# lucanest/Phyloformer

Hardware: AMD Instinct MI355X
Metric: alignments/sec, 60-leaf/500-site LG+GC-like MSAs, Phyloformer forward (pf.ckpt) (higher is better)
Workload: dtype f16x3-split MFMA (two fp16 limbs per operand, 3 passes), fp32 accumulate/residual

## Files before the change

### phyloformer_amd/csrc/pf_device.hip.h

```cpp
#pragma once
#include <hip/hip_runtime.h>
#include <stdint.h>

#include "pf_layout.h"

namespace pfk {

typedef float f32x4 __attribute__((ext_vector_type(4)));
typedef float f32x16 __attribute__((ext_vector_type(16)));
#if PF_F16
typedef _Float16 h16_t;
#define PF_MFMA(a, b, c) __builtin_amdgcn_mfma_f32_32x32x16_f16((a), (b), (c), 0, 0, 0)
#define PF_DOT2C "v_dot2c_f32_f16"
#define PF_CVT_PK "v_cvt_pk_f16_f32"
#define PF_NEG1_LO 0x0000bc00u
#define PF_NEG1_HI 0xbc000000u
#else
typedef __bf16 h16_t;
#define PF_MFMA(a, b, c) __builtin_amdgcn_mfma_f32_32x32x16_bf16((a), (b), (c), 0, 0, 0)
#define PF_DOT2C "v_dot2c_f32_bf16"
#define PF_CVT_PK "v_cvt_pk_bf16_f32"
#define PF_NEG1_LO 0x0000bf80u
#define PF_NEG1_HI 0xbf800000u
#endif
// ... 152 lines not shown
    r1 = fmaf((float)h2[1], -1.f, g1);
#else
    asm(PF_DOT2C_PRE PF_DOT2C " %0, %2, %4\n\t" PF_DOT2C " %1, %3, %4" PF_DOT2C_POST
                 : "+v"(r0), "+v"(r1) : "s"(PF_NEG1_LO), "s"(PF_NEG1_HI), "v"(hb));
#endif
    const h16x2 l2 = {(h16_t)r0, (h16_t)r1};
    hi_out = hb;
    lo_out = __builtin_bit_cast(unsigned, l2);
}
__device__ __forceinline__ void gelu_split_pair(float x0, float x1, unsigned& hi_out, unsigned& lo_out) {
    split_pair(gelu_scaled(x0), gelu_scaled(x1), hi_out, lo_out);
}
__device__ __forceinline__ void split8(const float* v, frag_t& hi, frag_t& lo) {
#if defined(PF_SPLIT_NODOT) || (PF_F16 && !defined(PF_SPLIT_DOT2C))
    u32x4 h, l;
#pragma unroll
    for (int k = 0; k < 4; ++k) {
        unsigned a, b;
        split_pair(v[2 * k], v[2 * k + 1], a, b);
        h[k] = a;
        l[k] = b;
    }
    hi = __builtin_bit_cast(frag_t, h);
    lo = __builtin_bit_cast(frag_t, l);
#else
    u32x4 h, l;
#pragma unroll
    for (int k = 0; k < 4; ++k) {
        const h16x2 h2 = {(h16_t)v[2 * k], (h16_t)v[2 * k + 1]};
        h[k] = __builtin_bit_cast(unsigned, h2);
    }
    float r0 = v[0], r1 = v[1], r2 = v[2], r3 = v[3], r4 = v[4], r5 = v[5], r6 = v[6], r7 = v[7];
    unsigned l0, l1, l2, l3;
    asm(
        PF_DOT2C " %4, %12, %14\n\t" PF_DOT2C " %5, %13, %14\n\t"
        PF_DOT2C " %6, %12, %15\n\t" PF_DOT2C " %7, %13, %15\n\t"
        PF_DOT2C " %8, %12, %16\n\t" PF_DOT2C " %9, %13, %16\n\t"
        PF_DOT2C " %10, %12, %17\n\t" PF_DOT2C " %11, %13, %17\n\ts_nop 1\n\t"
        PF_CVT_PK " %0, %4, %5\n\t" PF_CVT_PK " %1, %6, %7\n\t" PF_CVT_PK " %2, %8, %9\n\t" PF_CVT_PK " %3, %10, %11"
        : "=&v"(l0), "=&v"(l1), "=&v"(l2), "=&v"(l3),
          "+v"(r0), "+v"(r1), "+v"(r2), "+v"(r3), "+v"(r4), "+v"(r5), "+v"(r6), "+v"(r7)
        : "s"(PF_NEG1_LO), "s"(PF_NEG1_HI), "v"(h[0]), "v"(h[1]), "v"(h[2]), "v"(h[3]));
    l[0] = l0; l[1] = l1; l[2] = l2; l[3] = l3;
    hi = __builtin_bit_cast(frag_t, h);
    lo = __builtin_bit_cast(frag_t, l);
#endif
}
__device__ __forceinline__ void gelu_split8(const f32x16& acc, int base, frag_t& hi, frag_t& lo) {
    float g[8];
#pragma unroll
    for (int k = 0; k < 8; ++k) g[k] = gelu_scaled(acc[base + k]);
    split8(g, hi, lo);
}


__device__ __forceinline__ void mfma3(f32x16& acc, const frag_t& a_hi, const frag_t& a_lo,
                                      const frag_t& b_hi, const frag_t& b_lo, const bool flip = false) {
    if (!flip) {
        acc = PF_MFMA(a_hi, b_lo, acc);
        acc = PF_MFMA(a_hi, b_hi, acc);
        acc = PF_MFMA(a_lo, b_hi, acc);
    } else {
        acc = PF_MFMA(a_lo, b_hi, acc);
        acc = PF_MFMA(a_hi, b_hi, acc);
        acc = PF_MFMA(a_hi, b_lo, acc);
    }
}

__device__ __forceinline__ void mfma3_zero(f32x16& acc, const frag_t& a_hi, const frag_t& a_lo,
                                           const frag_t& b_hi, const frag_t& b_lo, const bool flip = false) {
    const f32x16 z = {0.f, 0.f, 0.f, 0.f, 0.f, 0.f, 0.f, 0.f, 0.f, 0.f, 0.f, 0.f, 0.f, 0.f, 0.f, 0.f};
    if (!flip) {
        acc = PF_MFMA(a_hi, b_lo, z);
        acc = PF_MFMA(a_hi, b_hi, acc);
        acc = PF_MFMA(a_lo, b_hi, acc);
    } else {
        acc = PF_MFMA(a_lo, b_hi, z);
        acc = PF_MFMA(a_hi, b_hi, acc);
        acc = PF_MFMA(a_hi, b_lo, acc);
    }
}

__device__ __forceinline__ void ln_pair(const float (&x)[32], float (&xn)[32]) {
    float s4[4] = {x[0], x[1], x[2], x[3]};
#pragma unroll
    for (int j = 4; j < 32; ++j) s4[j & 3] += x[j];
    const float mean = pair_sum((s4[0] + s4[1]) + (s4[2] + s4[3])) * (1.f / 64.f);
    float v4[4] = {0.f, 0.f, 0.f, 0.f};
#pragma unroll
    for (int j = 0; j < 32; ++j) {
        xn[j] = x[j] - mean;
        v4[j & 3] = fmaf(xn[j], xn[j], v4[j & 3]);
    }
    const float v = (v4[0] + v4[1]) + (v4[2] + v4[3]);
    const float rstd = __builtin_amdgcn_rsqf(pair_sum(v) * (1.f / 64.f) + LN_EPS);
#pragma unroll
    for (int j = 0; j < 32; ++j) xn[j] *= rstd;
}

typedef const f32x4 __attribute__((address_space(3)))* lds_f32x4_t;
__device__ __forceinline__ void load_acc_bias(f32x16& acc, lds_f32_t lds_bias_h) {
#pragma unroll
    for (int q4 = 0; q4 < 4; ++q4) {
        const f32x4 bb = *(lds_f32x4_t)(lds_bias_h + 8 * q4);
#pragma unroll
        for (int i = 0; i < 4; ++i) acc[4 * q4 + i] = bb[i];
    }
}

__device__ __forceinline__ void load_acc_bias(f32x16& acc, const float* lds_bias, int h) {
#pragma unroll
    for (int q4 = 0; q4 < 4; ++q4) {
        const f32x4 bb = *reinterpret_cast<const f32x4*>(lds_bias + 8 * q4 + 4 * h);
#pragma unroll
        for (int i = 0; i < 4; ++i) acc[4 * q4 + i] = bb[i];
    }
}

__device__ __forceinline__ frag_t zero_frag() {
    frag_t z;
#pragma unroll
    for (int i = 0; i < 8; ++i) z[i] = (h16_t)0.f;
    return z;
}

#ifndef PF_DEVICE_HELPERS_ONLY
struct MainArgs {
    float* x;
    float* qrow;
    const float* qcol;
    const frag_t* mfrag;
    const float* rq;
    const float* ctx;
    float* spart;
    float* outpart;
    const frag_t* wimg;
    const float* consts;
    const frag_t* wv_lo;
    const float* table;
    const uint8_t* idx;
    const int16_t* pair_i;
    const int16_t* pair_j;
    int B, N, P, Lloc;
    int flat;
    int nt_aln;
    int slots_aln;
    size_t trash_tok;
    int store_x_last;
    unsigned long long* prof;
    int ablate;
    float* sitemap;
    const float* w;
    const int* srep;
};

enum { MODE_FIRST = 0, MODE_MID = 1, MODE_LAST = 2, MODE_MID0 = 3, MODE_LAST_FOLD = 4 };

struct TilePos { int b, kt, r0, l0; };
template <bool FLAT>
__device__ __forceinline__ TilePos tile_pos(const MainArgs& a, int task, int ntiles) {
    TilePos q;
    q.b = task / a.nt_aln;
    q.kt = task - q.b * a.nt_aln;
    if (FLAT) { const int tok0 = q.kt * 32; q.r0 = tok0 / a.Lloc; q.l0 = tok0 - q.r0 * a.Lloc; }
    else { q.r0 = q.kt / ntiles; q.l0 = (q.kt - q.r0 * ntiles) * 32; }
    return q;
}
template <bool FLAT>
__device__ __forceinline__ TilePos tile_next(const MainArgs& a, TilePos q) {
    if (++q.kt == a.nt_aln) { q.b++; q.kt = 0; q.r0 = 0; q.l0 = 0; return q; }
    q.l0 += 32;
    if (q.l0 >= a.Lloc) { q.l0 = FLAT ? q.l0 - a.Lloc : 0; q.r0++; }
    return q;
}
struct LanePos { size_t tok0; int toff, l, nvalid, wrap; bool valid, in_r1; };
template <bool FLAT>
__device__ __forceinline__ LanePos lane_pos(const MainArgs& a, const TilePos& q, int t) {
    LanePos o;
    o.tok0 = ((size_t)q.b * a.P + q.r0) * a.Lloc + q.l0;
    const int left = FLAT ? a.P * a.Lloc - q.kt * 32 : a.Lloc - q.l0;
    o.nvalid = min(32, left);
    o.wrap = (FLAT && q.r0 + 1 < a.P) ? min(32, a.Lloc - q.l0) : 32;
    o.valid = t < o.nvalid;
    o.toff = min(t, o.nvalid - 1);
    o.in_r1 = o.toff >= o.wrap;
    o.l = q.l0 + o.toff - (o.in_r1 ? a.Lloc : 0);
    return o;
}
__device__ __forceinline__ void part_range(int flat, int pr, int nparts, int P, int L, int slots_aln, long* first, int* count) {
    if (!flat) { *first = (long)pr * nparts; *count = nparts; return; }
    const int b = pr / P, p = pr - b * P;
    const int k0 = (int)(((long)p * L) >> 5), k1 = (int)((((long)p + 1) * L - 1) >> 5);
    *first = (long)b * slots_aln + k0 + p;
    *count = k1 - k0 + 1;
}

template <int LO, int HI>
__device__ __forceinline__ void image_to_lds(const frag_t* src, unsigned char* smem) {
    static_assert(LO % 64 == 0 && HI % 64 == 0, "the image is copied in whole waves");
    const int wv = threadIdx.x >> 6, ln = threadIdx.x & 63;
#pragma unroll
    for (int k = 0; k < (HI - LO + MAIN_THREADS - 1) / MAIN_THREADS; ++k) {
        const int f0 = LO + k * MAIN_THREADS + wv * 64;
        if (f0 < HI) __builtin_amdgcn_global_load_lds(src + f0 + ln, smem + (size_t)f0 * 16, 16, 0, 0);
    }
}

template <int MODE, bool FLAT, bool SITEMAP = false, bool WEIGHTED = false>
__global__ void __launch_bounds__(MAIN_THREADS, MAIN_WAVES / 4) k_main(MainArgs a) {
    constexpr bool LAST = MODE == MODE_LAST || MODE == MODE_LAST_FOLD;
    constexpr bool FOLD = MODE == MODE_LAST_FOLD;
    static_assert(!SITEMAP || LAST, "the site map is the head's: last block only");
    static_assert(!WEIGHTED || (!SITEMAP && MODE != MODE_FIRST), "weighted launches: blocks' own modes, no site map");
    extern __shared__ __attribute__((aligned(16))) unsigned char smem[];
    lds_frag_t lw = (lds_frag_t)smem;
    lds_f32_t lc = (lds_f32_t)(smem + FRAG_END * 16);

    {
        const float cv = a.consts[min((int)threadIdx.x, CONST_LEN - 1)];
        if (FOLD) {
            image_to_lds<FRAG_W1, FRAG_W2>(a.wimg, smem);
            image_to_lds<FRAG_WO, FRAG_U + U_FRAGS>(a.wimg, smem);
        } else {
            image_to_lds<(MODE == MODE_FIRST) ? FRAG_WV : 0, LAST ? FRAG_WV : FRAG_END>(a.wimg, smem);
        }
        static_assert(CONST_LEN <= MAIN_THREADS, "one constant per thread");
        if (threadIdx.x < CONST_LEN) reinterpret_cast<float*>(smem + FRAG_END * 16)[threadIdx.x] = cv;
        asm volatile("s_waitcnt vmcnt(0)" ::: "memory");
    }
    __syncthreads();

    const int lane = threadIdx.x & 63;
    const int wave = __builtin_amdgcn_readfirstlane(threadIdx.x >> 6);
    const int t = lane & 31;
    const int h = lane >> 5;
    const int ntiles = (a.Lloc + 31) >> 5;
    const int ntasks = a.B * a.nt_aln;
    if (wave >= MAIN_WAVES / 2) __builtin_amdgcn_s_setprio(1);
    unsigned long long tacc[6] = {0, 0, 0, 0, 0, 0}, tprev = 0;
#define PF_TICK(k) do { if (a.prof) { const unsigned long long tn_ = __builtin_amdgcn_s_memtime(); tacc[k] += tn_ - tprev; tprev = tn_; } } while (0)
    if (a.prof) tprev = __builtin_amdgcn_s_memtime();
    lds_frag_t w1p = lw + FRAG_W1 + lane;
    lds_frag_t w2p = lw + FRAG_W2 + lane;
    lds_frag_t wop = lw + FRAG_WO + lane;
    lds_frag_t qkp = lw + FRAG_QK + h * 8 + (t & 7);
    lds_f32_t lch = lc + 4 * h;
    PF_OPAQUE(wop); PF_OPAQUE(qkp); PF_OPAQUE(lch);
    lds_frag_t wvp = wop + (FRAG_WV - FRAG_WO);
    lds_f32_t luh = (lds_f32_t)(smem + FRAG_U * 16) + 16 * h;

    {
        const int nwaves = gridDim.x * MAIN_WAVES;
#ifndef PF_RUN_MAX
#define PF_RUN_MAX 8
#endif
        const int run = max(1, min(PF_RUN_MAX, ntasks / (nwaves * 8)));
        int run0 = (blockIdx.x * MAIN_WAVES + wave) * run;
        const int task0 = run0, task1 = ntasks;
        TilePos cur = tile_pos<FLAT>(a, min(task0, ntasks - 1), ntiles);
        int frag_row = -1;
        frag_t mfr[4];
        f32x4 rqv = {0.f, 0.f, 0.f, 0.f};
        f32x4 px[8], pctx[8], pqr, pqc;
        int pri = 0, prj = 0;
        auto prefetch = [&](const TilePos& np) {
            const LanePos nl = lane_pos<FLAT>(a, np, t);
            const int ll = nl.l, pb = np.b;
            const size_t tk = nl.tok0 + nl.toff;
            if (MODE == MODE_MID0) {
                const uint8_t* ib = a.idx + (size_t)pb * a.N * a.Lloc + ll;
                const int pp = np.r0 + (nl.in_r1 ? 1 : 0);
                pri = residue(ib[(size_t)a.pair_i[pp] * a.Lloc]);
                prj = residue(ib[(size_t)a.pair_j[pp] * a.Lloc]);
            } else {
                const f32x4* xp = reinterpret_cast<const f32x4*>(a.x + tk * 64 + 4 * h);
#pragma unroll
                for (int g = 0; g < 8; ++g) px[g] = xp[2 * g];
            }
            pqr = *reinterpret_cast<const f32x4*>(a.qrow + tk * 4);
            pqc = *reinterpret_cast<const f32x4*>(a.qcol + (tk + (size_t)(long)(a.srep[(size_t)pb * a.Lloc + ll] - ll)) * 4);
            if (MODE != MODE_FIRST) {
                int hq = h;
                asm volatile("" : "+v"(hq));
                const f32x4* cp = reinterpret_cast<const f32x4*>(a.ctx + ((size_t)pb * a.Lloc + ll) * 64 + 4 * hq);
#pragma unroll
                for (int g = 0; g < 8; ++g) pctx[g] = cp[2 * g];
            }
        };
        if (MODE != MODE_FIRST && task0 < task1) prefetch(cur);

        for (int task = task0; task < task1;) {
            const int b = cur.b;
            const int row = b * a.P + cur.r0;
            int ntask = task + 1;
            TilePos nxt = tile_next<FLAT>(a, cur);
            if (ntask == run0 + run) {
                run0 += nwaves * run;
                ntask = run0;
                if (ntask < task1) nxt = tile_pos<FLAT>(a, ntask, ntiles);
            }
            const LanePos lp = lane_pos<FLAT>(a, cur, t);
            const bool straddle = lp.wrap < 32;
            int ai = 0, aj = 0;
            if (MODE == MODE_FIRST) { const int pp = cur.r0 + (lp.in_r1 ? 1 : 0); ai = a.pair_i[pp]; aj = a.pair_j[pp]; }
            auto load_mfr = [&](int r) {
                const frag_t* mf = a.mfrag + (size_t)r * 128 + t;
#pragma unroll
                for (int q = 0; q < 4; ++q) mfr[q] = mf[q * 32];
                typedef const f32x4 __attribute__((address_space(4)))* const_f32x4_t;
                rqv = *(const_f32x4_t)(unsigned long long)(a.rq + (size_t)__builtin_amdgcn_readfirstlane(r) * 4);
                frag_row = r;
            };
            if (MODE != MODE_FIRST && row != frag_row) load_mfr(row);
            const bool valid = lp.valid;
            const int lc_ = lp.l;
            const size_t tok = lp.tok0 + lp.toff;
            float x[32];
            float zh[4] = {0.f, 0.f, 0.f, 0.f};
            float wt = 1.f;
            if (WEIGHTED && LAST) wt = a.w[(size_t)b * a.Lloc + lc_];

            if (MODE == MODE_FIRST) {
                const int ri = residue(a.idx[((size_t)b * a.N + ai) * a.Lloc + lc_]);
                const int rj = residue(a.idx[((size_t)b * a.N + aj) * a.Lloc + lc_]);
                const f32x4* ti = reinterpret_cast<const f32x4*>(a.table + ri * 64 + 4 * h);
                const f32x4* tj = reinterpret_cast<const f32x4*>(a.table + rj * 64 + 4 * h);
#pragma unroll
                for (int g = 0; g < 8; ++g) {
                    f32x4 u = ti[2 * g], w = tj[2 * g];
#pragma unroll
                    for (int i = 0; i < 4; ++i) x[4 * g + i] = u[i] + w[i];
                }
            } else {
                if (MODE == MODE_MID0) {
                    const f32x4* ti = reinterpret_cast<const f32x4*>(a.table + pri * 64 + 4 * h);
                    const f32x4* tj = reinterpret_cast<const f32x4*>(a.table + prj * 64 + 4 * h);
#pragma unroll
                    for (int g = 0; g < 8; ++g) {
                        const f32x4 u = ti[2 * g], w = tj[2 * g];
#pragma unroll
                        for (int i = 0; i < 4; ++i) x[4 * g + i] = u[i] + w[i];
                    }
                } else {
#pragma unroll
                    for (int g = 0; g < 8; ++g)
#pragma unroll
                        for (int i = 0; i < 4; ++i) x[4 * g + i] = px[g][i];
                }
                PF_TICK(0);
                if (!(a.ablate & 8)) {
                    f32x16 ya[2];
#pragma unroll
                    for (int j = 0; j < 32; ++j) ya[j >> 4][j & 15] = x[j];
                    {
                        const f32x4 qr = pqr;
                        auto mix = [&](const bool mine) {
                            float v[8];
#pragma unroll
                            for (int i = 0; i < 4; ++i) v[i] = mine ? qr[i] * rqv[i] : 0.f;
                            v[4] = v[5] = mine ? 1.f : 0.f;
                            v[6] = v[7] = 0.f;
                            frag_t qb_hi, qb_lo;
                            split8(v, qb_hi, qb_lo);
#pragma unroll
                            for (int To = 0; To < 2; ++To) mfma3(ya[To], mfr[To * 2], mfr[To * 2 + 1], qb_hi, qb_lo, To == 1);
                        };
                        mix(h == 0 && !lp.in_r1);
                        if (straddle) {
                            load_mfr(row + 1);
                            mix(h == 0 && lp.in_r1);
                        }
                    }
                    {
                        const f32x4 qc = pqc * COLAPPLY_B_SCALE;
                        float o[32];
#pragma unroll
                        for (int g = 0; g < 8; ++g) {
                            const f32x4 u = pctx[g];
#pragma unroll
                            for (int i = 0; i < 4; ++i) o[4 * g + i] = u[i] * qc[g >> 1];
                        }
#pragma unroll
                        for (int s = 0; s < 4; ++s) {
                            frag_t ob_hi, ob_lo;
                            split8(&o[8 * s], ob_hi, ob_lo);
#pragma unroll
                            for (int To = 0; To < 2; ++To) {
                                lds_frag_t f = wop + ((To * 4 + s) * 2) * 64;
                                const frag_t a_hi = f[0], a_lo = f[64];
                                mfma3(ya[To], a_hi, a_lo, ob_hi, ob_lo, To == 1);
                            }
                        }
                    }
#pragma unroll
                    for (int j = 0; j < 32; ++j) x[j] = ya[j >> 4][j & 15];
                }

                PF_TICK(1);
                if (FOLD) {
#pragma unroll
                    for (int g = 0; g < 8; ++g) {
                        const f32x4 w4 = *(lds_f32x4_t)(lch + CONST_HW + 8 * g);
#pragma unroll
                        for (int i = 0; i < 4; ++i) zh[i] = fmaf(w4[i], x[4 * g + i], zh[i]);
                    }
                }
                if (FOLD && !(a.ablate & 16)) {
                    frag_t xb_hi[4], xb_lo[4];
                    {
                        float xn[32];
                        ln_pair(x, xn);
#pragma unroll
                        for (int s = 0; s < 4; ++s) split8(&xn[8 * s], xb_hi[s], xb_lo[s]);
                    }
                    if (ntask < task1) prefetch(nxt);
                    PF_TICK(2);
#pragma unroll 1
                    for (int T = 0; T < 8; ++T) {
                        f32x16 ha;
                        lds_frag_t f1 = w1p + T * 512;
                        lds_f32_t bp = lch + CONST_B1 + 32 * T;
                        lds_f32_t up = luh + 32 * T;
                        PF_OPAQUE(f1); PF_OPAQUE(bp); PF_OPAQUE(up);
                        load_acc_bias(ha, bp);
                        frag_t fh = f1[0], fl = f1[64];
#pragma unroll
                        for (int s = 0; s < 4; ++s) {
                            frag_t nh = fh, nl = fl;
                            if (s < 3) { nh = f1[(s + 1) * 128]; nl = f1[(s + 1) * 128 + 64]; }
                            mfma3(ha, fh, fl, xb_hi[s], xb_lo[s]);
                            fh = nh; fl = nl;
                        }
#pragma unroll
                        for (int q = 0; q < 4; ++q) {
                            const f32x4 u4 = *(lds_f32x4_t)(up + 4 * q);
#pragma unroll
                            for (int i = 0; i < 4; ++i) zh[i] = fmaf(u4[i], gelu_scaled(ha[4 * q + i]), zh[i]);
                        }
                    }
                    PF_TICK(3);
                } else if (!(a.ablate & 16)) {
                    frag_t xb_hi[4], xb_lo[4];
                    {
                        float xn[32];
                        ln_pair(x, xn);
#pragma unroll
                        for (int s = 0; s < 4; ++s) split8(&xn[8 * s], xb_hi[s], xb_lo[s]);
                    }
                    f32x16 oa[2];
                    load_acc_bias(oa[0], lch + CONST_B2);
                    load_acc_bias(oa[1], lch + CONST_B2 + 32);
#pragma unroll
                    for (int j = 0; j < 32; ++j) oa[j >> 4][j & 15] += x[j];
                    if (ntask < task1) prefetch(nxt);
                    PF_TICK(2);
#pragma unroll 1
                    for (int T = 0; T < 8; ++T) {
                        f32x16 ha;
                        lds_frag_t f1 = w1p + T * 512;
                        lds_frag_t f2 = w2p + T * 256;
                        lds_f32_t bp = lch + CONST_B1 + 32 * T;
                        PF_OPAQUE(f1); PF_OPAQUE(f2); PF_OPAQUE(bp);
                        load_acc_bias(ha, bp);
                        frag_t fh = f1[0], fl = f1[64];
#pragma unroll
                        for (int s = 0; s < 4; ++s) {
                            frag_t nh, nl;
                            if (s < 3) { nh = f1[(s + 1) * 128]; nl = f1[(s + 1) * 128 + 64]; }
                            else { nh = f2[0]; nl = f2[64]; }
                            mfma3(ha, fh, fl, xb_hi[s], xb_lo[s]);
                            fh = nh; fl = nl;
                        }
                        frag_t g_hi[2], g_lo[2];
                        gelu_split8(ha, 0, g_hi[0], g_lo[0]);
                        gelu_split8(ha, 8, g_hi[1], g_lo[1]);
#pragma unroll
                        for (int st = 0; st < 4; ++st) {
                            const int u = st >> 1, To = st & 1;
                            frag_t nh = fh, nl = fl;
                            if (st < 3) {
                                const int nu = (st + 1) >> 1, nTo = (st + 1) & 1;
                                nh = f2[(nTo * 32 + nu * 2) * 64];
                                nl = f2[(nTo * 32 + nu * 2) * 64 + 64];
                            }
                            mfma3(oa[To], fh, fl, g_hi[u], g_lo[u], To == 1);
                            fh = nh; fl = nl;
                        }
                    }
                    PF_TICK(3);
#pragma unroll
                    for (int j = 0; j < 32; ++j) x[j] = oa[j >> 4][j & 15];
                }
            }

            if (!LAST && !(a.ablate & 4)) {
                frag_t wl[8];
#pragma unroll
                for (int i = WVLO_LDS; i < 8; ++i) wl[i] = a.wv_lo[i * 64 + lane];
                if (WEIGHTED) wt = a.w[(size_t)b * a.Lloc + lc_];
                __builtin_amdgcn_sched_barrier(0);
                {
                    const size_t stok = valid ? tok : a.trash_tok + t;
                    f32x4* xo = reinterpret_cast<f32x4*>(a.x + stok * 64 + 4 * h);
#pragma unroll
                    for (int g = 0; g < 8; ++g) {
                        f32x4 u = {x[4 * g], x[4 * g + 1], x[4 * g + 2], x[4 * g + 3]};
                        xo[2 * g] = u;
                    }
                }
                if (a.ablate & 32) { cur = nxt; task = ntask; continue; }
                f32x16 va[3];
                {
                    float xn[32];
                    ln_pair(x, xn);
                    frag_t xb_hi[4], xb_lo[4];
#pragma unroll
                    for (int s = 0; s < 4; ++s) split8(&xn[8 * s], xb_hi[s], xb_lo[s]);
#pragma unroll
                    for (int s = 0; s < 4; ++s) {
                        const frag_t q_hi = qkp[(s * 2) * 16], q_lo = qkp[(s * 2 + 1) * 16];
                        if (s == 0) mfma3_zero(va[2], q_hi, q_lo, xb_hi[s], xb_lo[s]);
                        else mfma3(va[2], q_hi, q_lo, xb_hi[s], xb_lo[s]);
                    }
#pragma unroll
                    for (int s = 0; s < 4; ++s)
#pragma unroll
                        for (int T = 0; T < 2; ++T) {
                            const frag_t f_hi = wvp[(T * 4 + s) * 64];
                            const frag_t f_lo = T * 4 + s < WVLO_LDS ? wvp[(FRAG_WVLO - FRAG_WV) + (T * 4 + s) * 64] : wl[T * 4 + s];
                            if (s == 0) mfma3_zero(va[T], f_hi, f_lo, xb_hi[s], xb_lo[s], T == 1);
                            else mfma3(va[T], f_hi, f_lo, xb_hi[s], xb_lo[s], T == 1);
                        }
                }
#pragma unroll
                for (int r = 0; r < 4; ++r) va[2][r] += lc[CONST_BQK + 4 * h + r];
                float qk[4], ot[4];
#pragma unroll
                for (int i = 0; i < 4; ++i) qk[i] = elu1_fast(va[2][i]);
#pragma unroll
                for (int i = 0; i < 4; ++i) ot[i] = pair_other(qk[i], h);
                float qn[4], kn[4];
#pragma unroll
                for (int i = 0; i < 4; ++i) {
                    qn[i] = h ? ot[i] : qk[i];
                    kn[i] = h ? qk[i] : ot[i];
                }
                {
                    const size_t stok = valid ? tok : a.trash_tok + t;
                    f32x4 qs = {qn[0], qn[1], qn[2], qn[3]};
                    *reinterpret_cast<f32x4*>(a.qrow + stok * 4) = qs;
                }
                const long slot0 = (long)b * a.slots_aln + cur.kt + (FLAT ? cur.r0 : 0);
                for (int part = 0; part < (straddle ? 2 : 1); ++part) {
                    float* sp = a.spart + (size_t)(slot0 + part) * SROW;
                    const float vm = (valid && lp.in_r1 == (part == 1)) ? (WEIGHTED ? wt : 1.f) : 0.f;
                    float km[4];
#pragma unroll
                    for (int i = 0; i < 4; ++i) km[i] = kn[i] * vm;
                    {
                        float qk8[8];
#pragma unroll
                        for (int i = 0; i < 4; ++i) { qk8[i] = vm * qn[i]; qk8[4 + i] = km[i]; }
                        const float sqk = treduce8(qk8, t);
                        if (lane < 8) sp[64 + lane] = sqk;
                    }
                    {
                        float kv[32];
#pragma unroll
                        for (int j = 0; j < 32; ++j) kv[j] = km[j >> 3] * va[j >> 4][j & 15];
                        sp[kmap(t, h)] = treduce32(kv, t);
                    }
                }
            } else if (LAST) {
                float z = 0.f;
                if (FOLD) {
                    z = pair_sum((zh[0] + zh[1]) + (zh[2] + zh[3])) + lc[CONST_C0];
                } else {
#pragma unroll
                    for (int g = 0; g < 8; ++g) {
                        const f32x4 w4 = *(lds_f32x4_t)(lch + CONST_HW + 8 * g);
#pragma unroll
                        for (int i = 0; i < 4; ++i) z = fmaf(w4[i], x[4 * g + i], z);
                    }
                    z = pair_sum(z) + lc[CONST_HB];
                }
                const float spz = softplus20(z);
                const long slot0 = (long)b * a.slots_aln + cur.kt + (FLAT ? cur.r0 : 0);
                for (int part = 0; part < (straddle ? 2 : 1); ++part) {
                    const float so = half32_sum((valid && lp.in_r1 == (part == 1)) ? (WEIGHTED ? wt * spz : spz) : 0.f);
                    if (lane == 0) a.outpart[slot0 + part] = so;
                }
                if (SITEMAP && valid && h == 0) a.sitemap[lp.tok0 + lp.toff] = spz;
                if (!FOLD && a.store_x_last && valid) {
                    f32x4* xo = reinterpret_cast<f32x4*>(a.x + tok * 64 + 4 * h);
#pragma unroll
                    for (int g = 0; g < 8; ++g) {
                        f32x4 u = {x[4 * g], x[4 * g + 1], x[4 * g + 2], x[4 * g + 3]};
                        xo[2 * g] = u;
                    }
                }
            }
            PF_TICK(4);
            cur = nxt;
            task = ntask;
        }
    }
    if (a.prof && __builtin_amdgcn_mbcnt_hi(~0u, __builtin_amdgcn_mbcnt_lo(~0u, 0u)) == 0) {
#pragma unroll
        for (int k = 0; k < 6; ++k) atomicAdd(a.prof + k, tacc[k]);
    }
#undef PF_TICK
}

constexpr int EMBED_THREADS = 512;
constexpr int EMBED_LDS_BYTES = (PAIRTAB_ROWS * PAIRTAB_W + 22 * 64) * 4;
struct EmbedArgs {
    const uint8_t* idx;
    const int16_t* pair_i;
    const int16_t* pair_j;
    const float* ptab;
    const float* table;
    float* x;
    float* qrow;
    float* srow;
    int B, N, P, Lloc;
    unsigned* bad_idx;
    const float* w;
};

template <bool WEIGHTED = false>
__global__ void __launch_bounds__(EMBED_THREADS) k_embed(EmbedArgs a) {
    extern __shared__ __attribute__((aligned(16))) float esm[];
    float* tab = esm;
    float* emb = esm + PAIRTAB_ROWS * PAIRTAB_W;
    {
        constexpr int NV = PAIRTAB_ROWS * PAIRTAB_W / 4, FULL = NV / EMBED_THREADS;
        const f32x4* src = reinterpret_cast<const f32x4*>(a.ptab);
        f32x4* dst = reinterpret_cast<f32x4*>(tab);
        const int wv = threadIdx.x >> 6, ln = threadIdx.x & 63;
#pragma unroll
        for (int k = 0; k < FULL; ++k) {
            const int v0 = k * EMBED_THREADS + wv * 64;
            __builtin_amdgcn_global_load_lds(src + v0 + ln, tab + (size_t)v0 * 4, 16, 0, 0);
        }
        const int it = FULL * EMBED_THREADS + threadIdx.x;
        const f32x4 tail = src[min(it, NV - 1)];
        const f32x4* s2 = reinterpret_cast<const f32x4*>(a.table);
        f32x4* d2 = reinterpret_cast<f32x4*>(emb);
        static_assert(22 * 64 / 4 <= EMBED_THREADS, "one embedding vector per thread");
        const f32x4 ev = s2[min((int)threadIdx.x, 22 * 64 / 4 - 1)];
        if (it < NV) dst[it] = tail;
        if (threadIdx.x < 22 * 64 / 4) d2[threadIdx.x] = ev;
        asm volatile("s_waitcnt vmcnt(0)" ::: "memory");
    }
    __syncthreads();
    const int lane = threadIdx.x & 63, wave = threadIdx.x >> 6;
    const int sg = lane >> 4, cl = lane & 15;
    const int ntasks = a.B * a.P;
    for (int task = blockIdx.x * (EMBED_THREADS / 64) + wave; task < ntasks; task += gridDim.x * (EMBED_THREADS / 64)) {
        const int b = task / a.P, p = task - b * a.P;
        const uint8_t* ri = a.idx + ((size_t)b * a.N + a.pair_i[p]) * a.Lloc;
        const uint8_t* rj = a.idx + ((size_t)b * a.N + a.pair_j[p]) * a.Lloc;
        const size_t row0 = (size_t)task * a.Lloc;
        f32x4 acc = {0.f, 0.f, 0.f, 0.f}, acce = {0.f, 0.f, 0.f, 0.f};
        bool bad = false;
        auto fetch = [&](int blk) {
            const int l = min(blk * 64 + lane, a.Lloc - 1);
            const int ra = ri[l], rb = rj[l];
            bad |= max(ra, rb) >= NA;
            return residue(ra) * 22 + residue(rb);
        };
        auto fetch_w = [&](int blk) { return WEIGHTED ? a.w[(size_t)b * a.Lloc + min(blk * 64 + lane, a.Lloc - 1)] : 1.f; };
        const int nblk = (a.Lloc + 63) >> 6;
        int cur = fetch(0);
        float wcur = fetch_w(0);
        for (int blk = 0; blk < nblk; ++blk) {
            const int nxt = fetch(min(blk + 1, nblk - 1));
            const float wnxt = fetch_w(min(blk + 1, nblk - 1));
            const int lbase = blk * 64;
            const int nit = min(16, (a.Lloc - lbase + 3) >> 2);
            auto site = [&](int it, bool valid) {
                const int l = lbase + 4 * it + sg;
                const int rr = __shfl(cur, 4 * it + sg);
                const float* tr = tab + rr * PAIRTAB_W;
                const f32x4 s = *reinterpret_cast<const f32x4*>(tr + 4 * cl);
                const f32x4 e = *reinterpret_cast<const f32x4*>(tr + 64 + 4 * (cl & 1));
                const float wl = WEIGHTED ? __shfl(wcur, 4 * it + sg) : 1.f;
                if (valid) {
                    if (WEIGHTED) {
                        acc += wl * s;
                        acce += wl * e;
                    } else {
                        acc += s;
                        acce += e;
                    }
                    const size_t tok = row0 + l;
                    if (a.x) {
                        const int ra = rr / 22, rb = rr - 22 * ra;
                        const f32x4 xa = *reinterpret_cast<const f32x4*>(emb + ra * 64 + 4 * cl);
                        const f32x4 xb = *reinterpret_cast<const f32x4*>(emb + rb * 64 + 4 * cl);
                        *reinterpret_cast<f32x4*>(a.x + tok * 64 + 4 * cl) = xa + xb;
                    }
                    if (cl == 0) *reinterpret_cast<f32x4*>(a.qrow + tok * 4) = e;
                }
            };
            if (lbase + 64 <= a.Lloc) {
#pragma unroll 4
                for (int it = 0; it < 16; ++it) site(it, true);
            } else {
                for (int it = 0; it < nit; ++it) site(it, lbase + 4 * it + sg < a.Lloc);
            }
            cur = nxt;
            wcur = wnxt;
        }
#pragma unroll
        for (int i = 0; i < 4; ++i) {
            acc[i] += __shfl_xor(acc[i], 16);
            acc[i] += __shfl_xor(acc[i], 32);
            acce[i] += __shfl_xor(acce[i], 16);
            acce[i] += __shfl_xor(acce[i], 32);
        }
        if (sg == 0) {
            float* sr = a.srow + (size_t)task * SROW;
            *reinterpret_cast<f32x4*>(sr + 4 * cl) = acc;
            if (cl < 2) *reinterpret_cast<f32x4*>(sr + 64 + 4 * cl) = acce;
        }
        if (bad && a.bad_idx) *a.bad_idx = 1u;
    }
}

struct RowFinArgs {
    const float* srow;
    float* mrow;
    frag_t* mfrag;
    const float* woT;
    const float* bv;
    const float* bias;
    const float* bias_col;
    int npairs, nparts;
    float L_total;
    int flat, P, Lloc, slots_aln;
    int iters;
    float* rq;
    float a_scale, b_scale;
    const float* wst;
};

__global__ void __launch_bounds__(256) k_rowfin(RowFinArgs a) {
    __shared__ float ctx[4][64];
    __shared__ float mm[4][6][64];
    __shared__ float st[4][SROW];
    __shared__ float rqs[4][4];
    const int sub = threadIdx.x >> 6, c = threadIdx.x & 63;
    float wo[4][16];
#pragma unroll
    for (int hh = 0; hh < 4; ++hh)
#pragma unroll
        for (int d = 0; d < 16; ++d) wo[hh][d] = a.woT[(16 * hh + d) * 64 + c];
    const float bvc = a.bv[c], biasc = a.bias[c], biascol = a.bias_col[c];
    for (int it = 0; it < a.iters; ++it) {
    const int pr = (blockIdx.x * a.iters + it) * 4 + sub;
    const bool ok = pr < a.npairs;
    if (ok) {
        long first;
        int nparts;
        part_range(a.flat, pr, a.nparts, a.P, a.Lloc, a.slots_aln, &first, &nparts);
        const float* sp = a.srow + (size_t)first * SROW;
        const int c2 = 64 + (c & 7);
        float acc = 0.f, acc2 = 0.f;
        for (int i = 0; i < nparts; i += 8) {
            const float* q0 = sp + i * SROW;
            float v[8], w8[8];
#pragma unroll
            for (int q = 0; q < 8; ++q) {
                const bool on = i + q < nparts;
                v[q] = on ? q0[q * SROW + c] : 0.f;
                w8[q] = on ? q0[q * SROW + c2] : 0.f;
            }
#pragma unroll
            for (int q = 0; q < 8; ++q) { acc += v[q]; acc2 += w8[q]; }
        }
        st[sub][c] = acc;
        if (c < 8) st[sub][64 + c] = acc2;
    }
    __syncthreads();
    if (ok) {
        const float* s = st[sub];
        const int hh = c >> 4;
        const float sk = s[68 + hh];
        ctx[sub][c] = (s[c] + bvc * sk) / sk;
        if (c < 4) {
            const float* ws = a.wst ? a.wst + (size_t)(pr / a.P) * 4 : nullptr;
            const float r = (ws ? ws[0] : a.L_total) / s[64 + c];
            rqs[sub][c] = r;
            a.rq[(size_t)pr * 4 + c] = r * (ws ? ws[2] : a.b_scale);
        }
    }
    __syncthreads();
    if (ok) {
        float* m = a.mrow ? a.mrow + (size_t)pr * MROW : nullptr;
#pragma unroll
        for (int hh = 0; hh < 4; ++hh) {
            float acc = 0.f;
#pragma unroll
            for (int d = 0; d < 16; ++d) acc = fmaf(wo[hh][d], ctx[sub][16 * hh + d], acc);
            if (m) m[hh * 64 + c] = acc * rqs[sub][hh];
            mm[sub][hh][c] = acc * (a.wst ? a.wst[(size_t)(pr / a.P) * 4 + 3] : a.a_scale);
        }
        mm[sub][4][c] = biasc;
        mm[sub][5][c] = biascol;
    }
    __syncthreads();
    if (ok) {
        const int To = c >> 5, t = c & 31;
        float v[8];
#pragma unroll
        for (int i = 0; i < 8; ++i) v[i] = (i < 6) ? mm[sub][i][32 * To + t] : 0.f;
        frag_t hi, lo;
        split8(v, hi, lo);
        frag_t* mf = a.mfrag + (size_t)pr * MFRAG_PER_PAIR + To * 64 + t;
        mf[0] = hi;
        mf[32] = lo;
    }
    }
}

__global__ void k_rowsum(const float* spart, float* srow, int npairs, int nparts_, int flat, int P, int Lloc, int slots_aln) {
    const int i = blockIdx.x * blockDim.x + threadIdx.x;
    if (i >= npairs * SROW) return;
    const int pr = i / SROW, c = i - pr * SROW;
    long first;
    int nparts;
    part_range(flat, pr, nparts_, P, Lloc, slots_aln, &first, &nparts);
    const float* sp = spart + (size_t)first * SROW + c;
    float acc = 0.f;
    for (int k = 0; k < nparts; k += 8) {
        float v[8];
#pragma unroll
        for (int q = 0; q < 8; ++q) v[q] = k + q < nparts ? sp[(size_t)(k + q) * SROW] : 0.f;
#pragma unroll
        for (int q = 0; q < 8; ++q) acc += v[q];
    }
    srow[i] = acc;
}

__global__ void k_outsum(const float* outpart, float* out, int npairs, int nparts_, float inv_L_total, int flat, int P,
                         int Lloc, int slots_aln, const float* wst) {
    const int pr = blockIdx.x * blockDim.x + threadIdx.x;
    if (pr >= npairs) return;
    long first;
    int nparts;
    part_range(flat, pr, nparts_, P, Lloc, slots_aln, &first, &nparts);
    const float* sp = outpart + first;
    float acc = 0.f;
    for (int k = 0; k < nparts; k += 8) {
        float v[8];
#pragma unroll
        for (int q = 0; q < 8; ++q) v[q] = k + q < nparts ? sp[k + q] : 0.f;
#pragma unroll
        for (int q = 0; q < 8; ++q) acc += v[q];
    }
    out[pr] = acc * (wst ? wst[(size_t)(pr / P) * 4 + 1] : inv_L_total);
}

struct SiteClassArgs {
    const uint8_t* idx;
    int* srep;
    int* ulist;
    int* ucount;
    int N, Lloc, dedup;
};
constexpr int SC_THREADS = 1024, SC_MAX_SITES = 4096;
__global__ void __launch_bounds__(SC_THREADS) k_site_classes(SiteClassArgs a) {
    __shared__ __attribute__((aligned(16))) uint32_t hsh[SC_MAX_SITES];
    __shared__ int wsum[SC_THREADS / 64];
    const int b = blockIdx.x, tid = threadIdx.x, lane = tid & 63, wave = tid >> 6;
    const uint8_t* ib = a.idx + (size_t)b * a.N * a.Lloc;
    int* const srep = a.srep + (size_t)b * a.Lloc;
    int* const ulist = a.ulist + (size_t)b * a.Lloc;
    const bool dedup = a.dedup && a.Lloc <= SC_MAX_SITES;
    auto same_column = [&](int c, int l) {
        unsigned diff = 0;
#pragma unroll 8
        for (int n = 0; n < a.N; ++n) diff |= (unsigned)(ib[(size_t)n * a.Lloc + c] ^ ib[(size_t)n * a.Lloc + l]);
        return diff == 0;
    };
    if (dedup) {
        for (int l = tid; l < a.Lloc; l += SC_THREADS) {
            uint32_t hv = 0x811C9DC5u;
#pragma unroll 8
            for (int n = 0; n < a.N; ++n) hv = (hv ^ ib[(size_t)n * a.Lloc + l]) * 0x01000193u;
            hsh[l] = hv;
        }
        __syncthreads();
    }
    int base = 0;
    for (int l0 = 0; l0 < a.Lloc; l0 += SC_THREADS) {
        const int l = l0 + tid;
        int rep = l;
        if (dedup && l < a.Lloc) {
            const uint32_t mine = hsh[l];
            int cand = l;
            for (int c0 = 0; c0 < l && cand == l; c0 += 4) {
                const u32x4 v = *reinterpret_cast<const u32x4*>(hsh + c0);
#pragma unroll
                for (int i = 3; i >= 0; --i)
                    if (v[i] == mine && c0 + i < l) cand = c0 + i;
            }
            if (cand < l) {
                if (same_column(cand, l)) rep = cand;
                else
                    for (int c = cand + 1; c < l && rep == l; ++c)
                        if (hsh[c] == mine && same_column(c, l)) rep = c;
            }
        }
        const bool first = l < a.Lloc && rep == l;
        if (l < a.Lloc) srep[l] = rep;
        const unsigned long long m = __ballot(first);
        if (lane == 0) wsum[wave] = __popcll(m);
        __syncthreads();
        int before = 0, total = 0;
#pragma unroll
        for (int w = 0; w < SC_THREADS / 64; ++w) { const int n = wsum[w]; total += n; if (w < wave) before += n; }
        if (first) ulist[base + before + __popcll(m & ((1ull << lane) - 1ull))] = l;
        base += total;
        __syncthreads();
    }
    if (tid == 0) a.ucount[b] = base;
}

struct ColStatsArgs {
    const float* x;
    const float* qrow;
    const float* mrow;
    float* qcol;
    float* part;
    const float* wqk;
    const float* bqk;
    const float* brow;
    int B, P, Lloc, G, nchunks;
    int sub, S, fine;
    const float* table;
    const uint8_t* idx;
    const int16_t* pair_i;
    const int16_t* pair_j;
    int N;
    const int* ulist;
    const int* ucount;
};
constexpr int CPART = 4 * 64 + 8;

constexpr int CS_SLOT = 2 * 256 + 64;
#ifndef PF_CS_RING
#define PF_CS_RING 4
#endif
#ifndef PF_CS_MT
#define PF_CS_MT 16
#endif
template <bool EMBED, int RING, int MT>
#ifndef PF_CS_WAVES
#define PF_CS_WAVES 2
#endif
__global__ void __launch_bounds__(256, PF_CS_WAVES) k_colstats(ColStatsArgs a) {
    static_assert(!(EMBED && RING), "block 0 reads residue bytes, not x");
    static_assert(RING % 2 == 0, "pairs are consumed two at a time");
    static_assert(MT == 16 || MT == 8, "pair matrices are staged 16 or 8 at a time (runs are multiples of 8)");
    constexpr int LDS_MST = 2 * MT * MROW, LDS_RING = RING ? 4 * RING * CS_SLOT : 0, LDS_EMB = EMBED ? 22 * 64 : 0;
    constexpr int PIJ_CAP = 640;
    __shared__ __attribute__((aligned(16))) float lds_all[LDS_MST + LDS_RING + LDS_EMB + (EMBED ? PIJ_CAP : 0)];
    int bid = blockIdx.x;
    int run = 0;
    if (a.fine) { run = bid % a.S; bid /= a.S; }
    const int g = bid % a.G; bid /= a.G;
    const int chunk = bid % a.nchunks;
    const int b = bid / a.nchunks;
    const int nu = a.ucount[b];
    if (chunk * 32 >= nu) return;
    const int* const ul = a.ulist + (size_t)b * a.Lloc;
    float* const mst = lds_all;
    float* const xring = lds_all + LDS_MST;
    float* const emb = lds_all + LDS_MST + LDS_RING;
    int16_t* const pij = reinterpret_cast<int16_t*>(lds_all + LDS_MST + LDS_RING + LDS_EMB);
    if (EMBED) {
        constexpr int NV = 22 * 64 / 4;
        const f32x4* tsrc = reinterpret_cast<const f32x4*>(a.table);
        const int i0 = threadIdx.x, i1 = threadIdx.x + 256;
        static_assert(NV <= 2 * 256, "two vectors per thread cover the table");
        const f32x4 v0 = tsrc[min(i0, NV - 1)], v1 = tsrc[min(i1, NV - 1)];
        if (i0 < NV) reinterpret_cast<f32x4*>(emb)[i0] = v0;
        if (i1 < NV) reinterpret_cast<f32x4*>(emb)[i1] = v1;
    }
    const int lane = threadIdx.x & 63, wave = threadIdx.x >> 6;
    const int ts = lane >> 3, cl = lane & 7;
    const int per = (a.P + a.G - 1) / a.G;

    f32x2 w2[4][8];
#pragma unroll
    for (int o = 0; o < 8; o += 2)
#pragma unroll
        for (int q = 0; q < 2; ++q) {
            const f32x4 u0 = *reinterpret_cast<const f32x4*>(a.wqk + o * 64 + 8 * cl + 4 * q);
            const f32x4 u1 = *reinterpret_cast<const f32x4*>(a.wqk + (o + 1) * 64 + 8 * cl + 4 * q);
#pragma unroll
            for (int i = 0; i < 4; ++i) w2[o >> 1][4 * q + i] = f32x2{u0[i], u1[i]};
        }
    const float bj = a.bqk[cl];
    const f32x4 br0 = *reinterpret_cast<const f32x4*>(a.brow + 8 * cl), br1 = *reinterpret_cast<const f32x4*>(a.brow + 8 * cl + 4);
    const bool up1 = (cl & 2) != 0, up0 = (cl & 1) != 0;
    const int us = chunk * 32 + wave * 8 + ts;
    const bool lvalid = us < nu;
    const int l = ul[min(us, nu - 1)];
    const int lcl = l;
    const int gp0 = g * per, gp1 = min(a.P, gp0 + per);
    const int p0 = a.fine ? gp0 + run * a.sub : gp0, p1 = a.fine ? min(gp1, p0 + a.sub) : gp1;
    if (p0 >= p1) return;
    const float vmask = lvalid ? 1.f : 0.f;
    f32x2 z[4][4], zt[4][4];
// ... 342 lines not shown
```

### phyloformer_amd/csrc/pf_layout.h

```cpp
#pragma once

#ifndef PF_F16
#define PF_F16 1
#endif

namespace pfk {

constexpr int E = 64;
constexpr int NH = 4;
constexpr int HD = 16;
constexpr int FF = 256;
constexpr int NA = 22;
constexpr int SROW = 72;
constexpr int MROW = 4 * 64;
constexpr float LN_EPS = 1e-5f;

constexpr int FRAG_W1 = 0;
constexpr int FRAG_W2 = FRAG_W1 + 8 * 4 * 2 * 64;
constexpr int FRAG_WO = FRAG_W2 + 2 * 16 * 2 * 64;
constexpr int FRAG_WV = FRAG_WO + 2 * 4 * 2 * 64;
constexpr int FRAG_QK = FRAG_WV + 2 * 4 * 64;
#ifndef PF_WVLO_LDS
#define PF_WVLO_LDS 4
#endif
constexpr int WVLO_LDS = PF_WVLO_LDS;
constexpr int FRAG_WVLO = FRAG_QK + 4 * 2 * 16;
constexpr int FRAG_END = FRAG_WVLO + WVLO_LDS * 64;
constexpr int FRAG_U = FRAG_WV;
constexpr int U_FRAGS = FF * 4 / 16;
static_assert(FRAG_U + U_FRAGS <= FRAG_END, "the folded head fits the last block's tail");
constexpr int WVLO_FRAGS = 2 * 4 * 64;
constexpr int CONST_B1 = 0, CONST_B2 = 256, CONST_BQK = 320, CONST_HW = 328, CONST_HB = 392,
              CONST_C0 = 393, CONST_BOC = 400;
constexpr int CONST_LEN = 464;
constexpr int MAIN_LDS_BYTES = FRAG_END * 16 + CONST_LEN * 4;
constexpr int MFRAG_PER_PAIR = 2 * 2 * 32;

constexpr int MAIN_THREADS = 512;
constexpr int MAIN_WAVES = MAIN_THREADS / 64;

constexpr int PAIRTAB_ROWS = 22 * 22, PAIRTAB_W = 72;

}
```

### phyloformer_amd/csrc/pf_lib.hip

```cpp
#include <hip/hip_runtime.h>
#include <dlfcn.h>

#include <algorithm>
#include <cmath>
#include <cstdarg>
#include <cstdio>
#include <cstdlib>
#include <cstring>
#include <functional>
#include <map>
#include <mutex>
#include <string>
#include <type_traits>
#include <vector>

#include "../../include/phyloformer_amd.h"
#include "pf_device.hip.h"
#include "pf_mha.hip.h"
#include "pf_precise.hip.h"
#include "pf_generic.hip.h"
#include "pf_boot.hip.h"
#include "pf_sites.hip.h"
#include "pf_sitemap.hip.h"
#include "pf_sites_host.h"
// ... 15 lines not shown

namespace {

thread_local std::string g_create_error;

struct PfNcclId { char internal[128]; };
struct RcclApi {
    void* lib = nullptr;
    int (*GetUniqueId)(void*) = nullptr;
    int (*CommInitRank)(void**, int, PfNcclId, int) = nullptr;
    int (*AllReduce)(const void*, void*, size_t, int, int, void*, hipStream_t) = nullptr;
    int (*CommDestroy)(void*) = nullptr;
    const char* (*GetErrorString)(int) = nullptr;
};
RcclApi g_rccl;
std::string g_rccl_path;
int g_rccl_version = 0;
std::once_flag g_rccl_once;
std::string g_rccl_err;

bool load_rccl_once(std::string& err) {
    std::vector<std::string> names;
    if (const char* env = std::getenv("PF_RCCL_LIB")) names.push_back(env);
    else {
        if (const char* rocm = std::getenv("ROCM_PATH")) names.push_back(std::string(rocm) + "/lib/librccl.so.1");
        names.push_back("/opt/rocm/lib/librccl.so.1");
        names.push_back("librccl.so.1");
        names.push_back("librccl.so");
    }
    void* lib = nullptr;
    std::string tried;
    for (const std::string& n : names) {
        lib = dlopen(n.c_str(), RTLD_NOW | RTLD_LOCAL);
        if (lib) break;
        tried += (tried.empty() ? "" : ", ") + n;
    }
    if (!lib) { err = "cannot load librccl (tried " + tried + "): " + dlerror(); return false; }
    g_rccl.GetUniqueId = reinterpret_cast<int (*)(void*)>(dlsym(lib, "ncclGetUniqueId"));
    g_rccl.CommInitRank = reinterpret_cast<int (*)(void**, int, PfNcclId, int)>(dlsym(lib, "ncclCommInitRank"));
    g_rccl.AllReduce = reinterpret_cast<int (*)(const void*, void*, size_t, int, int, void*, hipStream_t)>(
        dlsym(lib, "ncclAllReduce"));
    g_rccl.CommDestroy = reinterpret_cast<int (*)(void*)>(dlsym(lib, "ncclCommDestroy"));
    g_rccl.GetErrorString = reinterpret_cast<const char* (*)(int)>(dlsym(lib, "ncclGetErrorString"));
    if (!g_rccl.GetUniqueId || !g_rccl.CommInitRank || !g_rccl.AllReduce || !g_rccl.CommDestroy) {
        err = "librccl is missing required symbols";
        return false;
    }
    Dl_info rinfo{}, hinfo{}, mine{};
    dladdr(reinterpret_cast<void*>(g_rccl.GetUniqueId), &rinfo);
    g_rccl_path = rinfo.dli_fname ? rinfo.dli_fname : "?";
    void* rccl_hip = dlsym(lib, "hipGetDeviceCount");
    if (rccl_hip && dladdr(rccl_hip, &hinfo) && dladdr(reinterpret_cast<void*>(&hipGetDeviceCount), &mine) &&
        hinfo.dli_fname && mine.dli_fname && std::strcmp(hinfo.dli_fname, mine.dli_fname) != 0) {
        err = std::string("librccl (") + g_rccl_path + ") is bound to the HIP runtime " + hinfo.dli_fname +
              " but this library uses " + mine.dli_fname + "; set PF_RCCL_LIB to the matching librccl";
        dlclose(lib);
        return false;
    }
    if (auto getv = reinterpret_cast<int (*)(int*)>(dlsym(lib, "ncclGetVersion"))) getv(&g_rccl_version);
    g_rccl.lib = lib;
    return true;
}
bool load_rccl(std::string& err) {
    std::call_once(g_rccl_once, [] { if (!load_rccl_once(g_rccl_err) && g_rccl_err.empty()) g_rccl_err = "librccl unavailable"; });
    if (g_rccl.lib) return true;
    err = g_rccl_err;
    return false;
}
constexpr int NCCL_FLOAT = 7, NCCL_DOUBLE = 8, NCCL_SUM = 0;

struct BlockDev {
    float* wimg = nullptr;
    float* consts = nullptr;
    float* wv_lo = nullptr;
    float* bqk_row = nullptr;
    float* row_woT = nullptr;
    float* row_bv = nullptr;
    float* row_bo = nullptr;
    float* col_bo = nullptr;
    float* col_wqk = nullptr;
    float* col_bqk = nullptr;
    float* col_wvT = nullptr;
    float* col_bv = nullptr;
};

struct ProfSlot { int kid; hipEvent_t a, b; };
const char* const KNAMES[] = {"embed", "rowfin", "colstats", "colfin", "main", "allreduce",
                              "mha_qkv", "mha_attn", "mha_out", "precise", "generic", "resample", "gather", "site_moments", "gather_taxa", "loo_stats",
                              "weight_sums", "place_stats", "tile_combine", "bme_pairs", "site_classes"};
enum { K_EMBED = 0, K_ROWFIN, K_COLSTATS, K_COLFIN, K_MAIN, K_ALLREDUCE, K_MHA_QKV, K_MHA_ATTN, K_MHA_OUT, K_PRECISE, K_GENERIC,
       K_RESAMPLE, K_GATHER, K_SITE_MOMENTS, K_GATHER_TAXA, K_LOO_STATS, K_WEIGHT_SUMS, K_PLACE_STATS, K_TILE_COMBINE, K_BME_PAIRS, K_SITE_CLASSES, K_COUNT };

struct F64Ends {
    const double* table = nullptr;
    const double *hw = nullptr, *hb = nullptr;
};

struct PreciseWeights {
    F64Ends ends;
    double* blob = nullptr;
    std::vector<pfp::AttnW> row, col;
    std::vector<pfp::FfnW> ffn;
};

struct GenericWeights {
    F64Ends ends;
    bool ready = false;
    std::vector<pfg::AttnW> row, col;
    std::vector<pfg::FfnW> ffn;
};

constexpr int64_t SUB_FLOATS_DEFAULT = (int64_t)1 << 22;

struct DeviceBuffer {
    void* p = nullptr; size_t cap = 0;
    explicit DeviceBuffer(std::vector<DeviceBuffer*>& all) { all.push_back(this); }
    DeviceBuffer(const DeviceBuffer&) = delete;
    int reserve(pf_handle* h, size_t bytes);
    void release() { if (p) hipFree(p); p = nullptr; cap = 0; }
};
template <class T> struct Buffer : DeviceBuffer {
    using DeviceBuffer::DeviceBuffer;
    operator T*() const { return static_cast<T*>(p); }
};

}

struct pf_handle {
    int device = 0;
    int n_blocks = 0;
    hipStream_t stream = nullptr;
    hipStream_t stream2 = nullptr;
    hipStream_t cur = nullptr;
    hipEvent_t ev_fork = nullptr, ev_join = nullptr;
    hipDeviceProp_t prop;
    std::string err;
    int64_t max_seqs = 200;
    bool profile = false;
    bool profile_main_only = false;
    bool debug_keep = false;
    int ablate = 0;
    unsigned long long* phase_prof = nullptr;
    bool phase_prof_last = false;
    bool head_fold = true;
    bool force_rccl = false;
    int64_t ws_limit_bytes = (int64_t)24 << 30;
    float* table = nullptr;
    float* pair_table = nullptr;
    bool embed_mfma = false;
    int colstats_fine = -1;
    bool colstats_ring = true;
    bool materialize_x0 = false;
    bool site_dedup = true;
    float* first_consts = nullptr;
    float* first_img = nullptr;
    std::vector<BlockDev> blk;
    std::vector<void*> owned;
    std::vector<DeviceBuffer*> buffers;
    int pair_n = -1;
    Buffer<int16_t> pair_i{buffers}, pair_j{buffers};
    Buffer<char> ws{buffers}, ws2{buffers};
    bool overlap = true;
    int reserve_cus = 8;
    Buffer<uint8_t> d_idx{buffers};
    Buffer<float> d_out{buffers};
    Buffer<uint8_t> d_rep{buffers};
    Buffer<int32_t> d_map{buffers};
    Buffer<float> d_smap{buffers}, d_se{buffers}, d_prof{buffers};
    Buffer<double> d_mpart{buffers};
    Buffer<char> d_sub{buffers};
    int64_t sub_floats = SUB_FLOATS_DEFAULT;
    pftile::Plan tiled_plan;
    pftile::Tables tiled_tab;
    Buffer<char> d_tiled_tab{buffers};
    Buffer<char> d_nj{buffers}, d_nj_io{buffers};
    int64_t nj_calls = 0;
    int64_t bionj_calls = 0;
    Buffer<char> d_delta_io{buffers};
    int64_t delta_calls = 0;
    bool delta_atomic = true;
    Buffer<char> d_bme{buffers};
    Buffer<float> d_bme_preds{buffers};
    int64_t bme_calls = 0;
    int64_t spr_calls = 0;
    bool spr_pairs_simple = false;
    int64_t spr_step_cap = 0;
    Buffer<char> d_sup{buffers}, d_sup_io{buffers};
    Buffer<uint8_t> d_sup_bad{buffers};
    int64_t sup_calls = 0;
    int64_t transfer_calls = 0;
    Buffer<char> d_con{buffers}, d_con_io{buffers};
    int64_t con_calls = 0;
    Buffer<float> d_w{buffers}, d_wst{buffers}, d_wtab{buffers};
    void* comm[2] = {nullptr, nullptr};
    int rank = 0, world = 1;
    int64_t coll_calls = 0;
    bool sharded_call = false;
    bool reducing = false;
    bool two_streams = true;
    std::vector<ProfSlot> pending;
    std::vector<hipEvent_t> free_events;
    int64_t prof_n[K_COUNT] = {0};
    double prof_ms[K_COUNT] = {0};
    std::map<std::string, std::vector<float>> taps;
    int tile_force = -1;
    int precise = -1;
    double recheck_above = 8.0;
    int64_t rechecked = 0;
    bool f16_ok = true;
    double f16_vmax_col = 0.0;
    char f16_why[160] = {0};
    bool precise_ffn_valu = false;
    PreciseWeights pw;
    Buffer<char> wsp{buffers};
    bool arch_generic = false;
    int generic = 0;
    pfg::Arch garch{};
    GenericWeights gw;
    std::vector<float> blob_copy;
    unsigned* bad_idx_host = nullptr;
    unsigned* bad_idx_dev = nullptr;
};

namespace {

int fail(pf_handle* h, int code, const char* fmt, ...) {
    char buf[512];
    va_list ap;
    va_start(ap, fmt);
    vsnprintf(buf, sizeof buf, fmt, ap);
    va_end(ap);
    if (h) h->err = buf; else g_create_error = buf;
    return code;
}

#define HIPCHK(h, call)                                                                 \
    do {                                                                                \
        hipError_t e_ = (call);                                                         \
        if (e_ != hipSuccess)                                                           \
            return fail((h), e_ == hipErrorOutOfMemory ? PF_ENOMEM : PF_EHIP, "%s: %s", \
                        #call, hipGetErrorString(e_));                                  \
    } while (0)

template <typename T>
int upload(pf_handle* h, const std::vector<T>& v, float** out) {
    void* p = nullptr;
    HIPCHK(h, hipMalloc(&p, v.size() * sizeof(T)));
    h->owned.push_back(p);
    HIPCHK(h, hipMemcpy(p, v.data(), v.size() * sizeof(T), hipMemcpyHostToDevice));
    *out = reinterpret_cast<float*>(p);
    return PF_OK;
}

int DeviceBuffer::reserve(pf_handle* h, size_t bytes) {
    if (p && bytes <= cap) return PF_OK;
    hipError_t e = hipSuccess;
    if (p) {
        e = hipStreamSynchronize(h->stream);
        if (e == hipSuccess && h->stream2) e = hipStreamSynchronize(h->stream2);
        release();
    }
    if (e == hipSuccess && (e = hipMalloc(&p, bytes ? bytes : 1)) != hipSuccess) p = nullptr;
    if (e != hipSuccess)
        return fail(h, e == hipErrorOutOfMemory ? PF_ENOMEM : PF_EHIP, "device buffer of %zu bytes: %s", bytes, hipGetErrorString(e));
    cap = bytes;
    return PF_OK;
}

struct F16Ranges { double hidden = 0, mbase = 0, vmax_col = 0, wmax = 0; };
void f16_note_attn(const std::vector<float>& wv, const std::vector<float>& bv, const float* wo, bool col, F16Ranges* r) {
    double vmax[E];
    for (int hd = 0; hd < E; ++hd) {
        double n2 = 0;
        for (int c = 0; c < E; ++c) { n2 += (double)wv[(size_t)hd * E + c] * wv[(size_t)hd * E + c]; r->wmax = std::max(r->wmax, std::fabs((double)wv[(size_t)hd * E + c])); }
        vmax[hd] = std::sqrt(n2) * 8.0 + std::fabs((double)bv[hd]);
        if (col) r->vmax_col = std::max(r->vmax_col, vmax[hd]);
    }
    for (int c = 0; c < E; ++c)
        for (int hh = 0; hh < NH; ++hh) {
            double m = 0;
            for (int d = 0; d < HD; ++d) { m += std::fabs((double)wo[(size_t)c * E + 16 * hh + d]) * vmax[16 * hh + d]; r->wmax = std::max(r->wmax, std::fabs((double)wo[(size_t)c * E + 16 * hh + d]) * (col ? COLAPPLY_A_SCALE : 1.0)); }
            if (!col) r->mbase = std::max(r->mbase, m);
        }
}
void f16_note_ffn(const std::vector<float>& w1a, const std::vector<float>& b1a, const std::vector<float>& w2s, F16Ranges* r) {
    for (int j = 0; j < FF; ++j) {
        double n2 = 0;
        for (int c = 0; c < E; ++c) { n2 += (double)w1a[(size_t)j * E + c] * w1a[(size_t)j * E + c]; r->wmax = std::max(r->wmax, std::fabs((double)w1a[(size_t)j * E + c])); }
        r->hidden = std::max(r->hidden, 2.0 * (std::sqrt(n2) * 8.0 + std::fabs((double)b1a[j])));
    }
    for (float v : w2s) r->wmax = std::max(r->wmax, std::fabs((double)v));
}
constexpr double F16_LIMIT = 60000.0;
void check_f16_ranges(pf_handle* h, const F16Ranges& r) {
    h->f16_vmax_col = r.vmax_col;
    const bool finite = std::isfinite(r.hidden) && std::isfinite(r.mbase) && std::isfinite(r.vmax_col) && std::isfinite(r.wmax);
    h->f16_ok = !PF_F16 || (finite && r.hidden < F16_LIMIT && r.mbase * 64.0 < F16_LIMIT && r.wmax < F16_LIMIT);
    if (!h->f16_ok)
        snprintf(h->f16_why, sizeof h->f16_why, "fp16 operand bounds: hidden %.3g, row-mix base %.3g, weights %.3g (limit %.0f)",
                 r.hidden, r.mbase * 64.0, r.wmax, F16_LIMIT);
}
bool f16_range_ok(const pf_handle* h, int N, int L_total) {
    if (!PF_F16) return true;
    const double P = (double)N * (N - 1) / 2;
    return h->f16_ok && P * h->f16_vmax_col * COLAPPLY_B_SCALE < F16_LIMIT && L_total <= (1 << 20);
}

int prepare_weights(pf_handle* h, const BlobView& view, uint64_t blob_len) {
    if ((uint64_t)view.len != blob_len)
        return fail(h, PF_EINVAL, "weight blob has %llu floats, expected %llu",
                    (unsigned long long)blob_len, (unsigned long long)view.len);
    std::vector<float> table((size_t)NA * E);
    build_embed_table(view, E, E, table.data());
    int rc = upload(h, table, &h->table);
    if (rc) return rc;

    const int nb = (int)view.ffn.size();
    h->blk.resize(nb);

    {
        std::vector<float> ptab;
        build_pair_table(table.data(), view.row[0], ptab);
        if ((rc = upload(h, ptab, &h->pair_table))) return rc;
    }
    F16Ranges ranges;
    std::vector<std::vector<float>> row_bqk(nb);
    std::vector<std::vector<uint16_t>> row_tail(nb);
    for (int k = 0; k < nb; ++k) {
        BlockDev& d = h->blk[k];
        const AttnHost& r = view.row[k];
        const AttnHost& c = view.col[k];
        std::vector<float> wq, bq, wk, bk, wv, bv;
        fold(r.wq, r.bq, r.g, r.b, NH, E, wq, bq);
        fold(r.wk, r.bk, r.g, r.b, NH, E, wk, bk);
        fold(r.wv, r.bv, r.g, r.b, E, E, wv, bv);
        f16_note_attn(wv, bv, r.wo, false, &ranges);
        for (float v : wq) ranges.wmax = std::max(ranges.wmax, std::fabs((double)v));
        for (float v : wk) ranges.wmax = std::max(ranges.wmax, std::fabs((double)v));
        row_tail[k].assign((size_t)(FRAG_END - FRAG_WV) * 8, 0);
        std::vector<uint16_t> wvlo((size_t)WVLO_FRAGS * 8);
        pack_row_stats(wv.data(), wq.data(), wk.data(), row_tail[k].data(), wvlo.data());
        std::copy(wvlo.begin(), wvlo.begin() + (size_t)WVLO_LDS * 64 * 8, row_tail[k].begin() + (size_t)(FRAG_WVLO - FRAG_WV) * 8);
        if ((rc = upload(h, wvlo, &d.wv_lo))) return rc;
        row_bqk[k].assign(8, 0.f);
        for (int i = 0; i < 4; ++i) { row_bqk[k][i] = bq[i]; row_bqk[k][4 + i] = bk[i]; }
        std::vector<float> woT((size_t)E * E);
        for (int cc = 0; cc < E; ++cc)
            for (int hd = 0; hd < E; ++hd) woT[(size_t)hd * E + cc] = r.wo[(size_t)cc * E + hd];
        if ((rc = upload(h, woT, &d.row_woT))) return rc;
        if ((rc = upload(h, bv, &d.row_bv))) return rc;
        if ((rc = upload(h, std::vector<float>(r.bo, r.bo + E), &d.row_bo))) return rc;
        if ((rc = upload(h, std::vector<float>(c.bo, c.bo + E), &d.col_bo))) return rc;
        std::vector<float> cwq, cbq, cwk, cbk, cwv, cbv;
        fold(c.wq, c.bq, c.g, c.b, NH, E, cwq, cbq);
        fold(c.wk, c.bk, c.g, c.b, NH, E, cwk, cbk);
        fold(c.wv, c.bv, c.g, c.b, E, E, cwv, cbv);
        f16_note_attn(cwv, cbv, c.wo, true, &ranges);
        std::vector<float> wqk((size_t)8 * E), bqk(8);
        std::copy(cwq.begin(), cwq.end(), wqk.begin());
        std::copy(cwk.begin(), cwk.end(), wqk.begin() + 4 * E);
        for (int i = 0; i < 4; ++i) { bqk[i] = cbq[i]; bqk[4 + i] = cbk[i]; }
        if ((rc = upload(h, wqk, &d.col_wqk))) return rc;
        if ((rc = upload(h, bqk, &d.col_bqk))) return rc;
        std::vector<float> wvT((size_t)E * E);
        for (int hd = 0; hd < E; ++hd)
            for (int cc = 0; cc < E; ++cc) wvT[(size_t)cc * E + hd] = cwv[(size_t)hd * E + cc];
        if ((rc = upload(h, wvT, &d.col_wvT))) return rc;
        if ((rc = upload(h, cbv, &d.col_bv))) return rc;
    }
    for (int k = 0; k < nb; ++k) {
        BlockDev& d = h->blk[k];
        const FfnHost& f = view.ffn[k];
        std::vector<float> w1f, b1f;
        fold(f.w1, f.b1, f.g, f.b, FF, E, w1f, b1f);
        const double alpha = std::sqrt(0.5 * 1.4426950408889634074);
        for (auto& v : w1f) v = (float)((double)v * alpha);
        for (auto& v : b1f) v = (float)((double)v * alpha);
        std::vector<float> w2s((size_t)E * FF);
        for (size_t i = 0; i < w2s.size(); ++i) w2s[i] = (float)((double)f.w2[i] / alpha * 0.5);
        f16_note_ffn(w1f, b1f, w2s, &ranges);
        std::vector<uint16_t> img((size_t)FRAG_END * 8);
        pack_frags(w1f.data(), FF, E, FF, img.data() + (size_t)FRAG_W1 * 8);
        pack_frags(w2s.data(), E, FF, E, img.data() + (size_t)FRAG_W2 * 8);
        pack_frags(view.col[k].wo, E, E, E, img.data() + (size_t)FRAG_WO * 8, COLAPPLY_A_SCALE);
        if (k + 1 < nb) std::copy(row_tail[k + 1].begin(), row_tail[k + 1].end(), img.begin() + (size_t)FRAG_WV * 8);
        float c0 = 0.f;
        if (k + 1 == nb) {
            float u[FF];
            fold_head(f.w2, f.b2, view.head_w, view.head_b[0], 1.0 / alpha * 0.5, u, &c0);
            std::memcpy(img.data() + (size_t)FRAG_U * 8, u, sizeof(u));
        }
        if ((rc = upload(h, img, &d.wimg))) return rc;
        std::vector<float> cst(CONST_LEN, 0.f);
        std::copy(b1f.begin(), b1f.end(), cst.begin() + CONST_B1);
        std::copy(f.b2, f.b2 + E, cst.begin() + CONST_B2);
        if (k + 1 < nb) std::copy(row_bqk[k + 1].begin(), row_bqk[k + 1].end(), cst.begin() + CONST_BQK);
        std::copy(view.head_w, view.head_w + E, cst.begin() + CONST_HW);
        cst[CONST_HB] = view.head_b[0];
        cst[CONST_C0] = c0;
        std::copy(view.col[k].bo, view.col[k].bo + E, cst.begin() + CONST_BOC);
        if ((rc = upload(h, cst, &d.consts))) return rc;
    }
    std::vector<float> cst0(CONST_LEN, 0.f);
    std::copy(row_bqk[0].begin(), row_bqk[0].end(), cst0.begin() + CONST_BQK);
    std::vector<uint16_t> img0((size_t)FRAG_END * 8, 0);
    std::copy(row_tail[0].begin(), row_tail[0].end(), img0.begin() + (size_t)FRAG_WV * 8);
    check_f16_ranges(h, ranges);
    if ((rc = upload(h, img0, &h->first_img))) return rc;
    return upload(h, cst0, &h->first_consts);
}

int ensure_pairs(pf_handle* h, int N) {
    if (h->pair_n == N) return PF_OK;
    const int P = N * (N - 1) / 2;
    std::vector<int16_t> pi(P), pj(P);
    int k = 0;
    for (int i = 0; i < N; ++i)
        for (int j = i + 1; j < N; ++j) { pi[k] = (int16_t)i; pj[k] = (int16_t)j; ++k; }
    h->pair_n = -1;
    int rc = h->pair_i.reserve(h, P * sizeof(int16_t));
    if (rc || (rc = h->pair_j.reserve(h, P * sizeof(int16_t)))) return rc;
    HIPCHK(h, hipMemcpyAsync(h->pair_i, pi.data(), P * sizeof(int16_t), hipMemcpyHostToDevice, h->stream));
    HIPCHK(h, hipMemcpyAsync(h->pair_j, pj.data(), P * sizeof(int16_t), hipMemcpyHostToDevice, h->stream));
    HIPCHK(h, hipStreamSynchronize(h->stream));
    h->pair_n = N;
    return PF_OK;
}

size_t align_up(size_t v, size_t a) { return (v + a - 1) / a * a; }

TilePlan tile_plan(const pf_handle* h, int P, int Lloc) { return tile_plan_core(P, Lloc, h->tile_force); }

struct Workspace {
    float *x, *qrow, *qcol, *srow, *mrow, *part, *ctx, *mfrag, *spart, *outpart, *rq;
    int *srep, *ulist, *ucount;
    int G;
    int sub, S, fine;
    int nparts() const { return fine ? G * S : G; }
};
constexpr int WS_BUFS = 12;

size_t workspace_bytes(const pf_handle* h, int B, int P, int Lloc, Workspace* w, size_t off[WS_BUFS]) {
    Lloc = std::max(Lloc, 1);
    const ColPlan c = colstats_plan_core(B, P, Lloc, h->colstats_fine);
    w->G = c.G; w->sub = c.sub; w->S = c.S; w->fine = c.fine;
    const int nparts = w->nparts();
    const size_t tok = (size_t)B * P * Lloc;
    size_t o = 0;
    off[0] = o; o = align_up(o + (tok + 32) * 64 * 4, 256);
    off[1] = o; o = align_up(o + (tok + 32) * 4 * 4, 256);
    off[2] = o; o = align_up(o + (tok + 32) * 4 * 4, 256);
    off[3] = o; o = align_up(o + (size_t)B * P * SROW * 4, 256);
    off[4] = o; o = align_up(o + (size_t)B * P * MROW * 4, 256);
    off[5] = o; o = align_up(o + (size_t)B * nparts * Lloc * CPART * 4, 256);
    off[6] = o; o = align_up(o + (size_t)B * Lloc * 64 * 4, 256);
    off[7] = o; o = align_up(o + (size_t)B * P * MFRAG_PER_PAIR * 16, 256);
    const size_t slots = (size_t)tile_plan(h, P, Lloc).slots_aln;
    off[8] = o; o = align_up(o + (size_t)B * slots * SROW * 4, 256);
    off[9] = o; o = align_up(o + (size_t)B * slots * 4, 256);
    off[10] = o; o = align_up(o + (size_t)B * P * 4 * 4, 256);
    off[11] = o; o = align_up(o + ((size_t)B * Lloc * 2 + B) * sizeof(int), 256);
    return o;
}
void carve_workspace(char* ws, const size_t off[WS_BUFS], Workspace* w, int B, int Lloc) {
    w->x = (float*)(ws + off[0]); w->qrow = (float*)(ws + off[1]);
    w->qcol = (float*)(ws + off[2]); w->srow = (float*)(ws + off[3]);
    w->mrow = (float*)(ws + off[4]); w->part = (float*)(ws + off[5]);
    w->ctx = (float*)(ws + off[6]);
    w->mfrag = (float*)(ws + off[7]);
    w->spart = (float*)(ws + off[8]); w->outpart = (float*)(ws + off[9]);
    w->rq = (float*)(ws + off[10]);
    const size_t nsite = (size_t)B * std::max(Lloc, 1);
    w->srep = (int*)(ws + off[11]); w->ulist = w->srep + nsite; w->ucount = w->ulist + nsite;
}

int ensure_workspace(pf_handle* h, int B, int P, int Lloc, Workspace* w, bool second = false) {
    size_t off[WS_BUFS];
    const size_t need = workspace_bytes(h, B, P, Lloc, w, off);
    Buffer<char>& ws = second ? h->ws2 : h->ws;
    if (const int rc = ws.reserve(h, need)) return rc;
    carve_workspace(ws, off, w, B, Lloc);
    return PF_OK;
}

hipEvent_t get_event(pf_handle* h) {
    if (!h->free_events.empty()) { hipEvent_t e = h->free_events.back(); h->free_events.pop_back(); return e; }
    hipEvent_t e;
    hipEventCreate(&e);
    return e;
}
struct ProfScope {
    pf_handle* h; int kid; hipEvent_t a{}, b{};
    bool on;
    ProfScope(pf_handle* h_, int kid_) : h(h_), kid(kid_) {
        on = h->profile && (!h->profile_main_only || kid_ == K_MAIN);
        if (on) { a = get_event(h); b = get_event(h); hipEventRecord(a, h->cur); }
    }
    ~ProfScope() {
        if (on) { hipEventRecord(b, h->cur); h->pending.push_back({kid, a, b}); }
    }
};
void drain_profile(pf_handle* h) {
    if (h->pending.empty()) return;
    hipStreamSynchronize(h->stream);
    if (h->stream2) hipStreamSynchronize(h->stream2);
    for (auto& s : h->pending) {
        float ms = 0.f;
        if (hipEventElapsedTime(&ms, s.a, s.b) == hipSuccess) { h->prof_n[s.kid]++; h->prof_ms[s.kid] += ms; }
        h->free_events.push_back(s.a);
        h->free_events.push_back(s.b);
    }
    h->pending.clear();
}

int save_tap(pf_handle* h, const std::string& name, const float* dptr, size_t n) {
    std::vector<float>& v = h->taps[name];
    v.resize(n);
    HIPCHK(h, hipStreamSynchronize(h->cur));
    HIPCHK(h, hipMemcpy(v.data(), dptr, n * sizeof(float), hipMemcpyDeviceToHost));
    return PF_OK;
}

int allreduce(pf_handle* h, void* buf, size_t count, int dtype = NCCL_FLOAT) {
    if (!h->sharded_call) return PF_OK;
    if (h->world <= 1 && !h->comm[0]) return PF_OK;
    if (!h->comm[0]) return fail(h, PF_ESTATE, "sharded forward on %d ranks needs pf_comm_init", h->world);
    ProfScope ps(h, K_ALLREDUCE);
    void* comm = h->comm[(h->cur == h->stream2 && h->stream2) ? 1 : 0];
    ++h->coll_calls;
    int rc = g_rccl.AllReduce(buf, buf, count, dtype, NCCL_SUM, comm, h->cur);
    if (rc != 0)
        return fail(h, PF_ERCCL, "ncclAllReduce failed: %s",
                    g_rccl.GetErrorString ? g_rccl.GetErrorString(rc) : "?");
    return PF_OK;
}

template <int MODE, bool SITEMAP = false, bool WEIGHTED = false>
int launch_main(pf_handle* h, const MainArgs& a, int kid) {
    const long ntasks = (long)a.B * a.nt_aln;
    const int cus = std::max(1, h->prop.multiProcessorCount - (h->reducing ? h->reserve_cus : 0));
    const int grid = (int)std::max<long>(1, std::min<long>(cus, (ntasks + MAIN_WAVES - 1) / MAIN_WAVES));
    ProfScope ps(h, kid);
    if (a.flat) hipLaunchKernelGGL((k_main<MODE, true, SITEMAP, WEIGHTED>), dim3(grid), dim3(MAIN_THREADS), MAIN_LDS_BYTES, h->cur, a);
    else hipLaunchKernelGGL((k_main<MODE, false, SITEMAP, WEIGHTED>), dim3(grid), dim3(MAIN_THREADS), MAIN_LDS_BYTES, h->cur, a);
    HIPCHK(h, hipGetLastError());
    return PF_OK;
}

struct RowStats { const float* p; int nparts; int flat; };
struct ShardRun {
    Workspace w;
    const uint8_t* d_idx;
    float* d_out;
    int B, N, P, Lloc, L_total;
    TilePlan tp;
    hipStream_t stream;
    RowStats rs;
    float* d_smap = nullptr;
    const float* d_w = nullptr;
    const float* d_wst = nullptr;
};

int zero_fill(pf_handle* h, float* p, size_t n) {
    HIPCHK(h, hipMemsetAsync(p, 0, n * sizeof(float), h->cur));
    return PF_OK;
}

MainArgs main_args(pf_handle* h, const ShardRun& r) {
    MainArgs m{};
    m.x = r.w.x; m.qrow = r.w.qrow; m.qcol = r.w.qcol;
    m.mfrag = reinterpret_cast<const frag_t*>(r.w.mfrag); m.rq = r.w.rq; m.ctx = r.w.ctx; m.spart = r.w.spart;
    m.outpart = r.w.outpart; m.table = h->table; m.idx = r.d_idx; m.pair_i = h->pair_i; m.pair_j = h->pair_j;
    m.B = r.B; m.N = r.N; m.P = r.P; m.Lloc = r.Lloc;
    m.flat = r.tp.flat; m.nt_aln = r.tp.nt_aln; m.slots_aln = r.tp.slots_aln;
    m.store_x_last = h->debug_keep ? 1 : 0;
    m.trash_tok = (size_t)r.B * r.P * r.Lloc;
    m.ablate = h->ablate;
    m.prof = h->phase_prof_last ? nullptr : h->phase_prof;
    m.w = r.d_w;
    m.srep = r.w.srep;
    return m;
}

bool x0_on_the_fly(const pf_handle* h) {
    return !h->materialize_x0 && !h->embed_mfma && h->n_blocks > 1;
}

int launch_site_classes(pf_handle* h, const uint8_t* d_idx, int B, int N, int Lloc, int* srep, int* ulist, int* ucount) {
    if (!Lloc) return PF_OK;
    SiteClassArgs a{d_idx, srep, ulist, ucount, N, Lloc, h->site_dedup ? 1 : 0};
    ProfScope ps(h, K_SITE_CLASSES);
    hipLaunchKernelGGL(k_site_classes, dim3(B), dim3(SC_THREADS), 0, h->cur, a);
    HIPCHK(h, hipGetLastError());
    return PF_OK;
}

int phase_first(pf_handle* h, const ShardRun& r) {
    if (!r.Lloc) return zero_fill(h, r.w.srow, (size_t)r.B * r.P * SROW);
    int rc;
    if (h->embed_mfma) {
        MainArgs m = main_args(h, r);
        m.wimg = reinterpret_cast<const frag_t*>(h->first_img); m.consts = h->first_consts;
        m.wv_lo = reinterpret_cast<const frag_t*>(h->blk[0].wv_lo);
        rc = launch_main<MODE_FIRST>(h, m, K_EMBED);
        if (rc) return rc;
    } else {
        float* x0 = (x0_on_the_fly(h) && !h->debug_keep) ? nullptr : r.w.x;
        EmbedArgs e{r.d_idx, h->pair_i, h->pair_j, h->pair_table, h->table, x0, r.w.qrow, r.w.srow,
                    r.B, r.N, r.P, r.Lloc, h->bad_idx_dev, r.d_w};
        const int ntasks = r.B * r.P, wpb = EMBED_THREADS / 64;
        const int grid = std::max(1, std::min(h->prop.multiProcessorCount, (ntasks + wpb - 1) / wpb));
        ProfScope ps(h, K_EMBED);
        if (r.d_w) hipLaunchKernelGGL(k_embed<true>, dim3(grid), dim3(EMBED_THREADS), EMBED_LDS_BYTES, h->cur, e);
        else hipLaunchKernelGGL(k_embed<false>, dim3(grid), dim3(EMBED_THREADS), EMBED_LDS_BYTES, h->cur, e);
        HIPCHK(h, hipGetLastError());
    }
    if (h->debug_keep) return save_tap(h, "x0", r.w.x, (size_t)r.B * r.P * r.Lloc * 64);
    return PF_OK;
}

int tiles_of(int Lloc) { return (Lloc + 31) / 32; }

int launch_rowsum(pf_handle* h, const ShardRun& r, RowStats* rs) {
    if (rs->p == r.w.srow) return PF_OK;
    const int n = r.B * r.P * SROW;
    if (!r.Lloc) { *rs = RowStats{r.w.srow, 1, 0}; return zero_fill(h, r.w.srow, n); }
    ProfScope ps(h, K_ROWFIN);
    hipLaunchKernelGGL(k_rowsum, dim3((n + 255) / 256), dim3(256), 0, h->cur, rs->p, r.w.srow, r.B * r.P, rs->nparts,
                       rs->flat, r.P, r.Lloc, r.tp.slots_aln);
    HIPCHK(h, hipGetLastError());
    *rs = RowStats{r.w.srow, 1, 0};
    return PF_OK;
}

int launch_outsum(pf_handle* h, const ShardRun& r) {
    const int n = r.B * r.P;
    if (!r.Lloc) return zero_fill(h, r.d_out, n);
    ProfScope ps(h, K_ROWFIN);
    const TilePlan& tp = r.tp;
    hipLaunchKernelGGL(k_outsum, dim3((n + 255) / 256), dim3(256), 0, h->cur, r.w.outpart, r.d_out, n,
                       tiles_of(r.Lloc), 1.0f / (float)r.L_total, tp.flat, r.P, r.Lloc, tp.slots_aln, r.d_wst);
    HIPCHK(h, hipGetLastError());
    return PF_OK;
}

RowStats main_stats(const ShardRun& r) { return RowStats{r.w.spart, tiles_of(r.Lloc), r.tp.flat}; }

RowStats first_stats(pf_handle* h, const ShardRun& r) {
    return h->embed_mfma ? main_stats(r) : RowStats{r.w.srow, 1, 0};
}

int phase_block(pf_handle* h, const ShardRun& r, int k, RowStats rs) {
    if (!r.Lloc) return PF_OK;
    const BlockDev& d = h->blk[k];
    const Workspace& w = r.w;
    const int B = r.B, P = r.P, Lloc = r.Lloc;
    int rc;
    if (h->debug_keep) {
        if ((rc = launch_rowsum(h, r, &rs))) return rc;
        if ((rc = save_tap(h, "srow" + std::to_string(k), rs.p, (size_t)B * P * SROW))) return rc;
    }
    {
        RowFinArgs a{rs.p, w.mrow, reinterpret_cast<frag_t*>(w.mfrag),
                     d.row_woT, d.row_bv, d.row_bo, d.col_bo,
                     B * P, rs.nparts, (float)r.L_total, rs.flat, P, Lloc, r.tp.slots_aln, 1};
        const int groups = (B * P + 3) / 4;
        a.iters = std::max(1, std::min(16, groups / (4 * 8 * std::max(1, h->prop.multiProcessorCount))));
        a.rq = w.rq;
        a.b_scale = 1.f;
        for (long lim = 16384; lim < (long)r.L_total && a.b_scale > 1.f / 256.f; lim *= 2) a.b_scale *= 0.5f;
        a.a_scale = 1.f / a.b_scale;
        a.wst = r.d_wst;
        ProfScope ps(h, K_ROWFIN);
        hipLaunchKernelGGL(k_rowfin, dim3((groups + a.iters - 1) / a.iters), dim3(256), 0, h->cur, a);
        HIPCHK(h, hipGetLastError());
    }
    {
        ColStatsArgs a{w.x, w.qrow, w.mrow, w.qcol, w.part, d.col_wqk, d.col_bqk, d.row_bo, B, P, Lloc, w.G, (Lloc + 31) / 32,
                       w.sub, w.S, w.fine, h->table, r.d_idx, h->pair_i, h->pair_j, r.N, w.ulist, w.ucount};
        ProfScope ps(h, K_COLSTATS);
        const unsigned nblk = (unsigned)(B * a.nchunks * w.nparts());
        if (k == 0 && x0_on_the_fly(h))
            hipLaunchKernelGGL((k_colstats<true, 0, 16>), dim3(nblk), dim3(256), 0, h->cur, a);
        else if (h->colstats_ring)
            hipLaunchKernelGGL((k_colstats<false, PF_CS_RING, PF_CS_MT>), dim3(nblk), dim3(256), 0, h->cur, a);
        else
            hipLaunchKernelGGL((k_colstats<false, 0, 16>), dim3(nblk), dim3(256), 0, h->cur, a);
        HIPCHK(h, hipGetLastError());
    }
    {
        ColFinArgs a{w.part, w.ctx, d.col_wvT, d.col_bv, B, Lloc, w.G, (float)P, P, w.sub, w.S, w.fine, w.srep};
        ProfScope ps(h, K_COLFIN);
        hipLaunchKernelGGL(k_colfin, dim3(B * Lloc), dim3(COLFIN_THREADS), 0, h->cur, a);
        HIPCHK(h, hipGetLastError());
    }
    if (h->debug_keep) {
        if ((rc = save_tap(h, "ctx" + std::to_string(k), w.ctx, (size_t)B * Lloc * 64))) return rc;
        if ((rc = save_tap(h, "mrow" + std::to_string(k), w.mrow, (size_t)B * P * MROW))) return rc;
    }
    MainArgs m = main_args(h, r);
    m.wimg = reinterpret_cast<const frag_t*>(d.wimg);
    m.consts = d.consts;
    if (k + 1 < h->n_blocks) {
        m.wv_lo = reinterpret_cast<const frag_t*>(h->blk[k + 1].wv_lo);
        const bool first = k == 0 && x0_on_the_fly(h);
        if (r.d_w) rc = first ? launch_main<MODE_MID0, false, true>(h, m, K_MAIN) : launch_main<MODE_MID, false, true>(h, m, K_MAIN);
        else rc = first ? launch_main<MODE_MID0>(h, m, K_MAIN) : launch_main<MODE_MID>(h, m, K_MAIN);
        if (rc) return rc;
    } else {
        m.wv_lo = nullptr;
        if (h->phase_prof_last) m.prof = h->phase_prof;
        m.sitemap = r.d_smap;
        if (!h->head_fold) {
            if ((rc = r.d_w      ? launch_main<MODE_LAST, false, true>(h, m, K_MAIN)
                      : r.d_smap ? launch_main<MODE_LAST, true>(h, m, K_MAIN) : launch_main<MODE_LAST>(h, m, K_MAIN))) return rc;
        } else {
            if ((rc = r.d_w      ? launch_main<MODE_LAST_FOLD, false, true>(h, m, K_MAIN)
                      : r.d_smap ? launch_main<MODE_LAST_FOLD, true>(h, m, K_MAIN) : launch_main<MODE_LAST_FOLD>(h, m, K_MAIN)))
                return rc;
            if (h->debug_keep) {
                MainArgs md = m;
                md.outpart = w.spart;
                md.prof = nullptr;
                if ((rc = r.d_w ? launch_main<MODE_LAST, false, true>(h, md, K_MAIN) : launch_main<MODE_LAST>(h, md, K_MAIN))) return rc;
            }
        }
    }
    if (h->debug_keep && (rc = save_tap(h, "x" + std::to_string(k + 1), w.x, (size_t)B * P * Lloc * 64))) return rc;
    return PF_OK;
}

bool reduces_now(const pf_handle* h) { return h->sharded_call && (h->world > 1 || h->comm[0]); }
bool empty_rank_call(const pf_handle* h, int Lloc) { return Lloc == 0 && reduces_now(h); }

int halves_of(const pf_handle* h, int B) {
    if (B < 2 || h->debug_keep) return 1;
    if (reduces_now(h)) return h->overlap ? 2 : 1;
    return h->two_streams ? 2 : 1;
}

int ensure_second_stream(pf_handle* h) {
    if (h->stream2) return PF_OK;
    HIPCHK(h, hipStreamCreateWithFlags(&h->stream2, hipStreamNonBlocking));
    HIPCHK(h, hipEventCreateWithFlags(&h->ev_fork, hipEventDisableTiming));
    HIPCHK(h, hipEventCreateWithFlags(&h->ev_join, hipEventDisableTiming));
    return PF_OK;
}

struct ForwardScope {
    pf_handle* h;
    ForwardScope(pf_handle* h_, bool reduces) : h(h_) { h->reducing = reduces; }
    ~ForwardScope() { h->cur = h->stream; h->reducing = false; }
};

template <class Reduce>
int schedule(pf_handle* h, ShardRun* runs, size_t nruns, Reduce reduce) {
    ShardRun* const end = runs + nruns;
    int rc;
    for (ShardRun* r = runs; r != end; ++r) {
        h->cur = r->stream;
        if ((rc = launch_site_classes(h, r->d_idx, r->B, r->N, r->Lloc, r->w.srep, r->w.ulist, r->w.ucount))) return rc;
        if ((rc = phase_first(h, *r))) return rc;
        r->rs = first_stats(h, *r);
    }
    for (int k = 0; k < h->n_blocks; ++k) {
        if ((rc = reduce(false))) return rc;
        for (ShardRun* r = runs; r != end; ++r) {
            h->cur = r->stream;
            if ((rc = phase_block(h, *r, k, r->rs))) return rc;
            r->rs = main_stats(*r);
        }
    }
    for (ShardRun* r = runs; r != end; ++r) {
        h->cur = r->stream;
        if ((rc = launch_outsum(h, *r))) return rc;
    }
    return reduce(true);
}

int forward_chunk(pf_handle* h, const uint8_t* d_idx, int B, int N, int Lloc, int L_total, float* d_out,
                  float* d_smap = nullptr, const float* d_w = nullptr, const float* d_wst = nullptr) {
    const int P = N * (N - 1) / 2;
    const bool reduces = reduces_now(h);
    const int nh = halves_of(h, B);
    int rc = ensure_pairs(h, N);
    if (rc) return rc;
    ShardRun r[2]{};
    int b0 = 0;
    for (int i = 0; i < nh; ++i) {
        const int nb = (nh == 2) ? (i == 0 ? (B + 1) / 2 : B / 2) : B;
        r[i] = ShardRun{{}, d_idx + (size_t)b0 * N * Lloc, d_out + (size_t)b0 * P, nb, N, P, Lloc, L_total,
                        tile_plan(h, P, Lloc), h->stream, {}};
        if (d_smap) r[i].d_smap = d_smap + (size_t)b0 * P * Lloc;
        if (d_w) { r[i].d_w = d_w + (size_t)b0 * Lloc; r[i].d_wst = d_wst + (size_t)b0 * pfw::WST; }
        if ((rc = ensure_workspace(h, nb, P, Lloc, &r[i].w, i == 1))) return rc;
        b0 += nb;
    }
    ForwardScope scope(h, reduces);
    if (nh == 2) {
        if ((rc = ensure_second_stream(h))) return rc;
        r[1].stream = h->stream2;
        HIPCHK(h, hipEventRecord(h->ev_fork, h->stream));
        HIPCHK(h, hipStreamWaitEvent(h->stream2, h->ev_fork, 0));
    }
    auto reduce = [&](bool site_sums) -> int {
        if (!reduces) return PF_OK;
        for (ShardRun* q = r; q != r + nh; ++q) {
            h->cur = q->stream;
            if (!site_sums && (rc = launch_rowsum(h, *q, &q->rs))) return rc;
            if ((rc = allreduce(h, site_sums ? q->d_out : q->w.srow, (size_t)q->B * P * (site_sums ? 1 : SROW)))) return rc;
        }
        return PF_OK;
    };
    if ((rc = schedule(h, r, nh, reduce))) return rc;
    if (nh == 2) {
        HIPCHK(h, hipEventRecord(h->ev_join, h->stream2));
        HIPCHK(h, hipStreamWaitEvent(h->stream, h->ev_join, 0));
    }
    return PF_OK;
}

struct ShardStage {
    struct Shard { int Lloc; const uint8_t* d_idx; };
    pf_handle* h;
    const bool keep;
    std::vector<void*> allocs;
    std::vector<Shard> shards;
    explicit ShardStage(pf_handle* h_) : h(h_), keep(h_->debug_keep) { h->debug_keep = false; }
    ShardStage(const ShardStage&) = delete;
    ~ShardStage() {
        hipStreamSynchronize(h->stream);
        for (void* p : allocs) hipFree(p);
        h->debug_keep = keep;
    }
    void* alloc(size_t bytes) {
        void* p = nullptr;
        if (hipMalloc(&p, bytes ? bytes : 1) != hipSuccess) return nullptr;
        allocs.push_back(p);
        return p;
    }
    int upload(const uint8_t* idx, int B, int N, int L, int nshards) {
        const int step = (L + nshards - 1) / nshards;
        for (int s = 0; s < nshards; ++s) {
            const int lo = std::min(s * step, L), hi = std::min((s + 1) * step, L);
            if (hi <= lo) continue;
            const int Lloc = hi - lo;
            uint8_t* di = (uint8_t*)alloc((size_t)B * N * Lloc);
            if (!di) return fail(h, PF_ENOMEM, "shard workspace allocation failed");
            std::vector<uint8_t> local((size_t)B * N * Lloc);
            for (int b = 0; b < B; ++b)
                for (int n = 0; n < N; ++n)
                    std::memcpy(&local[((size_t)b * N + n) * Lloc], &idx[((size_t)b * N + n) * L + lo], Lloc);
            if (hipMemcpy(di, local.data(), local.size(), hipMemcpyHostToDevice) != hipSuccess) return fail(h, PF_EHIP, "idx upload failed");
            shards.push_back({Lloc, di});
        }
        return PF_OK;
    }
};

int make_room(pf_handle* h, bool f64, size_t need) {
    const size_t budget = std::max(need, (size_t)h->ws_limit_bytes);
    if (f64 && h->wsp) { HIPCHK(h, hipStreamSynchronize(h->stream)); h->wsp.release(); }
    if (h->ws.cap + h->ws2.cap + (f64 ? need : h->wsp.cap) <= budget) return PF_OK;
    HIPCHK(h, hipStreamSynchronize(h->stream));
    if (h->stream2) HIPCHK(h, hipStreamSynchronize(h->stream2));
    if (!f64) {
        h->wsp.release();
        if (h->ws.cap + h->ws2.cap <= budget) return PF_OK;
    }
    h->ws.release(); h->ws2.release();
    return PF_OK;
}

#include "pf_f64_host.hip.h"

int check_dims(pf_handle* h, int B, int N, int Lloc, int L_total) {
    if (!h) return PF_EINVAL;
    if (h->n_blocks == 0) return fail(h, PF_ESTATE, "handle was created without Phyloformer weights (pf_create_bare)");
    if (B < 1 || N < 2 || Lloc < (empty_rank_call(h, Lloc) ? 0 : 1) || L_total < std::max(Lloc, 1))
        return fail(h, PF_EINVAL, "bad dimensions B=%d N=%d L=%d (L_total=%d)", B, N, Lloc, L_total);
    if (h->max_seqs > 0 && N > h->max_seqs)
        return fail(h, PF_EINVAL, "n_seqs must be smaller or equal to %lld (or pre-compute a larger global_seq2pair)",
                    (long long)h->max_seqs);
    if (N > 32767) return fail(h, PF_EINVAL, "n_seqs %d exceeds the pair-table index range", N);
    return PF_OK;
}

size_t chunk_bytes(const pf_handle* h, int cb, int P, int Lloc) {
    size_t off[WS_BUFS];
    const int nh = halves_of(h, cb);
    const int b0 = nh == 2 ? (cb + 1) / 2 : cb, b1 = nh == 2 ? cb / 2 : 0;
    size_t total = 0;
    for (int nb : {b0, b1}) {
        if (nb < 1) continue;
        Workspace w;
        total += workspace_bytes(h, nb, P, Lloc, &w, off);
    }
    return total;
}

int chunk_batch(pf_handle* h, int B, int P, int Lloc, size_t extra = 0) {
    B = (int)std::min<long>(B, std::max<long>(1, 0x7fffffffL / std::max(1, tile_plan(h, P, Lloc).nt_aln) - 1));
    auto fits = [&](int cb) { return chunk_bytes(h, cb, P, Lloc) + (size_t)cb * extra <= (size_t)h->ws_limit_bytes; };
    if (B <= 1 || fits(B)) return std::max(B, 1);
    int lo = 1, hi = B;
    while (hi - lo > 1) {
        const int mid = lo + (hi - lo) / 2;
        if (fits(mid)) lo = mid; else hi = mid;
    }
    return lo;
}

template <class Go>
int launch_on_stream(pf_handle* h, int kid, const char* name, Go&& go) {
    h->cur = h->stream;
    ProfScope ps(h, kid);
    const hipError_t e = go();
    if (e != hipSuccess) return fail(h, PF_EHIP, "%s launch failed: %s", name, hipGetErrorString(e));
    return PF_OK;
}

int launch_weight_sums(pf_handle* h, const float* d_w, int B, int L, const float** d_wst) {
    int rc = h->d_wst.reserve(h, (size_t)B * pfw::WST * sizeof(float));
    if (rc) return rc;
    *d_wst = h->d_wst;
    return launch_on_stream(h, K_WEIGHT_SUMS, "k_weight_sums",
                            [&] { return pfw::launch_weight_sums(h->stream, d_w, h->d_wst, B, L, h->bad_idx_dev + 2); });
}

int check_weighted_handle(pf_handle* h) {
    if (h->world > 1)
        return fail(h, PF_ESTATE, "weighted forwards are not site-sharded: this handle's communicator has %d ranks (use a "
                                  "handle without a communicator)", h->world);
    if (h->embed_mfma) return fail(h, PF_ESTATE, "option embed_mfma has no weighted kernel (set it to 0 for weighted forwards)");
    return PF_OK;
}

int check_weights(pf_handle* h, const float* w, size_t rows, int K, const char* what) {
    const int64_t at = pfweights::first_bad_weight(w, rows * (size_t)K);
    if (at >= 0)
        return fail(h, PF_EINVAL, "weight %g of %s %lld, position %lld is negative or not finite", (double)w[at], what,
                    (long long)(at / K), (long long)(at % K));
    for (size_t r = 0; r < rows; ++r) {
        const float W = pfweights::weight_sum(w + r * (size_t)K, K);
        if (!(W > 0.f && W <= 3.402823466e38f))
            return fail(h, PF_EINVAL, "the weights of %s %zu sum to %g: W must be positive and finite", what, r, (double)W);
    }
// ... 1139 lines not shown

int pf_abi_version(void) { return PF_ABI_VERSION; }

uint64_t pf_blob_len(int32_t n_blocks, int32_t n_heads, int32_t embed_dim) {
    return read_blob(nullptr, n_blocks, embed_dim, n_heads).len;
}

static int open_device(int device, pf_handle** out) {
    int ndev = 0;
    hipError_t e = hipGetDeviceCount(&ndev);
    if (e != hipSuccess || ndev == 0)
        return fail(nullptr, PF_EHIP, "no HIP device available (%s); there is no CPU fallback",
                    e != hipSuccess ? hipGetErrorString(e) : "device count is 0");
    if (device < 0 || device >= ndev) return fail(nullptr, PF_EINVAL, "device %d out of range (have %d)", device, ndev);
    pf_handle* h = new pf_handle();
    if (const char* e = getenv("PF_TWO_STREAMS")) h->two_streams = atoi(e) != 0;
    if (getenv("PF_ROW_TILES")) h->tile_force = 0;
    if (getenv("PF_FLAT_TILES")) h->tile_force = 1;
    if (const char* v = getenv("PF_COLSTATS_RING")) h->colstats_ring = atoi(v) != 0;
    h->device = device;
    int rc = PF_OK;
    do {
        if ((e = hipSetDevice(device)) != hipSuccess) { rc = fail(nullptr, PF_EHIP, "hipSetDevice: %s", hipGetErrorString(e)); break; }
        if ((e = hipGetDeviceProperties(&h->prop, device)) != hipSuccess) { rc = fail(nullptr, PF_EHIP, "hipGetDeviceProperties: %s", hipGetErrorString(e)); break; }
        if (std::string(h->prop.gcnArchName).rfind("gfx950", 0) != 0) {
            rc = fail(nullptr, PF_EHIP, "device %d is %s; this library is built for gfx950 only", device, h->prop.gcnArchName);
            break;
        }
        if ((e = hipStreamCreateWithFlags(&h->stream, hipStreamNonBlocking)) != hipSuccess) { rc = fail(nullptr, PF_EHIP, "hipStreamCreate: %s", hipGetErrorString(e)); break; }
        h->cur = h->stream;
        if ((e = hipHostMalloc((void**)&h->bad_idx_host, 3 * sizeof(unsigned), hipHostMallocMapped | hipHostMallocCoherent)) != hipSuccess ||
            (e = hipHostGetDevicePointer((void**)&h->bad_idx_dev, h->bad_idx_host, 0)) != hipSuccess) {
            rc = fail(nullptr, PF_EHIP, "hipHostMalloc (residue flag): %s", hipGetErrorString(e));
            break;
        }
        h->bad_idx_host[0] = h->bad_idx_host[1] = h->bad_idx_host[2] = 0u;
        const struct { const void* fn; int bytes; } big_lds[] = {
            {reinterpret_cast<const void*>(&k_main<MODE_FIRST, false>), MAIN_LDS_BYTES},
            {reinterpret_cast<const void*>(&k_main<MODE_MID, false>), MAIN_LDS_BYTES},
            {reinterpret_cast<const void*>(&k_main<MODE_MID0, false>), MAIN_LDS_BYTES},
            {reinterpret_cast<const void*>(&k_main<MODE_LAST, false>), MAIN_LDS_BYTES},
            {reinterpret_cast<const void*>(&k_main<MODE_LAST_FOLD, false>), MAIN_LDS_BYTES},
            {reinterpret_cast<const void*>(&k_main<MODE_FIRST, true>), MAIN_LDS_BYTES},
            {reinterpret_cast<const void*>(&k_main<MODE_MID, true>), MAIN_LDS_BYTES},
            {reinterpret_cast<const void*>(&k_main<MODE_MID0, true>), MAIN_LDS_BYTES},
            {reinterpret_cast<const void*>(&k_main<MODE_LAST, true>), MAIN_LDS_BYTES},
            {reinterpret_cast<const void*>(&k_main<MODE_LAST_FOLD, true>), MAIN_LDS_BYTES},
            {reinterpret_cast<const void*>(&k_main<MODE_LAST, false, true>), MAIN_LDS_BYTES},
            {reinterpret_cast<const void*>(&k_main<MODE_LAST_FOLD, false, true>), MAIN_LDS_BYTES},
            {reinterpret_cast<const void*>(&k_main<MODE_LAST, true, true>), MAIN_LDS_BYTES},
            {reinterpret_cast<const void*>(&k_main<MODE_LAST_FOLD, true, true>), MAIN_LDS_BYTES},
            {reinterpret_cast<const void*>(&k_main<MODE_MID, false, false, true>), MAIN_LDS_BYTES},
            {reinterpret_cast<const void*>(&k_main<MODE_MID0, false, false, true>), MAIN_LDS_BYTES},
            {reinterpret_cast<const void*>(&k_main<MODE_LAST, false, false, true>), MAIN_LDS_BYTES},
            {reinterpret_cast<const void*>(&k_main<MODE_LAST_FOLD, false, false, true>), MAIN_LDS_BYTES},
            {reinterpret_cast<const void*>(&k_main<MODE_MID, true, false, true>), MAIN_LDS_BYTES},
            {reinterpret_cast<const void*>(&k_main<MODE_MID0, true, false, true>), MAIN_LDS_BYTES},
            {reinterpret_cast<const void*>(&k_main<MODE_LAST, true, false, true>), MAIN_LDS_BYTES},
            {reinterpret_cast<const void*>(&k_main<MODE_LAST_FOLD, true, false, true>), MAIN_LDS_BYTES},
            {reinterpret_cast<const void*>(&k_embed<false>), EMBED_LDS_BYTES},
            {reinterpret_cast<const void*>(&k_embed<true>), EMBED_LDS_BYTES},
        };
        for (const auto& k : big_lds)
            if ((e = hipFuncSetAttribute(k.fn, hipFuncAttributeMaxDynamicSharedMemorySize, k.bytes)) != hipSuccess) {
                rc = fail(nullptr, PF_EHIP, "hipFuncSetAttribute: %s", hipGetErrorString(e));
                break;
            }
        if (rc) break;
    } while (0);
    if (rc) { pf_destroy(h); return rc; }
    *out = h;
    return PF_OK;
}

int pf_create_bare(int device, pf_handle_t** out) {
    if (!out) return fail(nullptr, PF_EINVAL, "null argument");
    *out = nullptr;
    return open_device(device, out);
}

int pf_create(const pf_weights_t* w, int device, pf_handle_t** out) {
    if (!w || !out || !w->blob) return fail(nullptr, PF_EINVAL, "null argument");
    *out = nullptr;
    if (!generic_arch_ok(w))
        return fail(nullptr, PF_EINVAL,
                    "unsupported architecture: n_blocks=%d n_heads=%d embed_dim=%d n_alphabet=%d "
                    "(n_alphabet must be 22, n_blocks 1..64, embed_dim must be 1..256 and divisible by n_heads)",
                    w->n_blocks, w->n_heads, w->embed_dim, w->n_alphabet);
    if (w->blob_len != pf_blob_len(w->n_blocks, w->n_heads, w->embed_dim))
        return fail(nullptr, PF_EINVAL, "weight blob has %llu floats, expected %llu",
                    (unsigned long long)w->blob_len,
                    (unsigned long long)pf_blob_len(w->n_blocks, w->n_heads, w->embed_dim));
    pf_handle* h = nullptr;
    int rc = open_device(device, &h);
    if (rc) return rc;
    h->n_blocks = w->n_blocks;
    h->garch = pfg::make_arch(w->embed_dim, w->n_heads);
    const BlobView bv = read_blob(w->blob, w->n_blocks, w->embed_dim, w->n_heads);
    if (w->embed_dim == E && w->n_heads == NH) {
        rc = prepare_weights(h, bv, w->blob_len);
        if (!rc) rc = prepare_precise_weights(h, bv, &h->pw);
        if (!rc) {
            try { h->blob_copy.assign(w->blob, w->blob + w->blob_len); }
            catch (const std::bad_alloc&) { rc = fail(h, PF_ENOMEM, "out of host memory copying the weights"); }
        }
    } else {
        h->arch_generic = true;
        rc = prepare_generic_weights(h, bv);
    }
    if (rc) g_create_error = h->err;
    if (rc) { pf_destroy(h); return rc; }
    *out = h;
    return PF_OK;
}

int pf_destroy(pf_handle_t* h) {
    if (!h) return PF_OK;
    hipSetDevice(h->device);
    if (h->stream) hipStreamSynchronize(h->stream);
    if (h->stream2) hipStreamSynchronize(h->stream2);
    for (void*& c : h->comm) if (c && g_rccl.CommDestroy) { g_rccl.CommDestroy(c); c = nullptr; }
    for (auto& s : h->pending) { hipEventDestroy(s.a); hipEventDestroy(s.b); }
    for (auto e : h->free_events) hipEventDestroy(e);
    for (void* p : h->owned) hipFree(p);
    for (DeviceBuffer* b : h->buffers) b->release();
    if (h->stream2) hipStreamDestroy(h->stream2);
    if (h->ev_fork) hipEventDestroy(h->ev_fork);
    if (h->ev_join) hipEventDestroy(h->ev_join);
    if (h->stream) hipStreamDestroy(h->stream);
    if (h->bad_idx_host) hipHostFree(h->bad_idx_host);
    delete h;
    return PF_OK;
}

const char* pf_last_error(const pf_handle_t* h) { return h ? h->err.c_str() : g_create_error.c_str(); }

int pf_set_option(pf_handle_t* h, const char* key, int64_t value) {
    if (!h || !key) return PF_EINVAL;
    const std::string k(key);
    if (k == "max_seqs") h->max_seqs = value;
    else if (k == "profile") { drain_profile(h); h->profile = value != 0; h->profile_main_only = value == 2; }
    else if (k == "debug_keep") h->debug_keep = value != 0;
    else if (k == "embed_mfma") h->embed_mfma = value != 0;
    else if (k == "colstats_fine") h->colstats_fine = value < 0 ? -1 : (value != 0);
    else if (k == "materialize_x0") h->materialize_x0 = value != 0;
    else if (k == "overlap") h->overlap = value != 0;
    else if (k == "two_streams") h->two_streams = value != 0;
    else if (k == "reserve_cus") h->reserve_cus = (int)std::max<int64_t>(0, std::min<int64_t>(value, 128));
    else if (k == "ablate") h->ablate = (int)value;
    else if (k == "head_fold") h->head_fold = value != 0;
    else if (k == "force_rccl") h->force_rccl = value != 0;
    else if (k == "colstats_ring") h->colstats_ring = value != 0;
    else if (k == "site_dedup") h->site_dedup = value != 0;
    else if (k == "precise") h->precise = value < 0 ? -1 : (value != 0);
    else if (k == "recheck_above") h->recheck_above = value > 0 ? (double)value : 0.0;
    else if (k == "precise_ffn_valu") h->precise_ffn_valu = value != 0;
    else if (k == "generic") {
        if (h->arch_generic && !value)
            return fail(h, PF_EINVAL, "embed_dim %d / n_heads %d runs on the generic kernels only (option generic cannot be 0)",
                        h->garch.E, h->garch.NH);
        h->generic = value != 0;
    }
    else if (k == "phase_prof") {
        if (value && !h->phase_prof) { HIPCHK(h, hipMalloc((void**)&h->phase_prof, 64)); h->owned.push_back(h->phase_prof); }
        if (h->phase_prof) HIPCHK(h, hipMemset(h->phase_prof, 0, 64));
        if (!value) h->phase_prof = nullptr;
        h->phase_prof_last = value == 2;
    }
    else if (k == "ws_limit_mb") h->ws_limit_bytes = value << 20;
    else if (k == "spr_pairs_simple") h->spr_pairs_simple = value != 0;
    else if (k == "delta_atomic") h->delta_atomic = value != 0;
    else if (k == "spr_step_cap") h->spr_step_cap = value > 0 ? value : 0;
    else if (k == "sub_floats") h->sub_floats = value > 0 ? value : SUB_FLOATS_DEFAULT;
    else return fail(h, PF_EINVAL, "unknown option '%s'", key);
    return PF_OK;
}

int pf_forward(pf_handle_t* h, const uint8_t* idx, int32_t B, int32_t N, int32_t L, float* out) {
    if (!h) return PF_EINVAL;
    return forward_host_impl(h, idx, B, N, 0, L, L, out);
}

int pf_resample_sites_device(pf_handle_t* h, const uint8_t* d_src, int32_t B, int32_t N, int32_t L, int32_t r_begin, int32_t R,
                             uint64_t seed, uint8_t* d_dst) {
    if (!h) return PF_EINVAL;
    if (!d_src || !d_dst) return fail(h, PF_EINVAL, "null buffer");
    if (B < 1 || N < 1 || L < 1 || R < 1 || r_begin < 0)
        return fail(h, PF_EINVAL, "bad dimensions B=%d N=%d L=%d r_begin=%d R=%d", B, N, L, r_begin, R);
    size_t n = 0;
    if (!mul_size((size_t)B, (size_t)R, (size_t)N * L, &n))
        return fail(h, PF_EINVAL, "B=%d x R=%d replicates of %d x %d overflow the address space", B, R, N, L);
    HIPCHK(h, hipSetDevice(h->device));
    return launch_resample(h, d_src, B, N, L, r_begin, R, seed, d_dst);
}

int pf_bootstrap(pf_handle_t* h, const uint8_t* idx, int32_t B, int32_t N, int32_t L, int32_t R, uint64_t seed, float* out) {
    if (!h) return PF_EINVAL;
    return bootstrap_impl(h, idx, B, N, L, R, seed, out);
}

int pf_window_count(int32_t L, int32_t W, int32_t step) {
    const int n = pfsites::window_count(L, W, step);
    return n < 0 ? PF_EINVAL : n;
}

int pf_window_start(int32_t L, int32_t W, int32_t step, int32_t s) {
    const int st = pfsites::window_start(L, W, step, s);
    return st < 0 ? PF_EINVAL : st;
}

int pf_gather_sites_device(pf_handle_t* h, const uint8_t* d_src, int32_t B, int32_t N, int32_t L, const int32_t* d_sites,
                           const int32_t* d_start, int32_t S, int32_t K, uint8_t* d_dst) {
    if (!h) return PF_EINVAL;
    if (!d_src || !d_dst) return fail(h, PF_EINVAL, "null buffer");
    if (!d_sites == !d_start) return fail(h, PF_EINVAL, "exactly one of d_sites (table) and d_start (affine) must be given");
    if (B < 1 || N < 1 || L < 1 || S < 1 || K < 1 || K > L)
        return fail(h, PF_EINVAL, "bad dimensions B=%d N=%d L=%d S=%d K=%d (1 <= K <= L)", B, N, L, S, K);
    size_t n = 0;
    if (!mul_size((size_t)B, (size_t)S, (size_t)N * K, &n) || !mul_size((size_t)S, (size_t)K, sizeof(int32_t), &n))
        return fail(h, PF_EINVAL, "B=%d x S=%d site sets of %d x %d overflow the address space", B, S, N, K);
    HIPCHK(h, hipSetDevice(h->device));
    return launch_gather(h, d_src, B, N, L, d_sites, d_start, 0, S, K, d_dst);
}

int pf_forward_sites(pf_handle_t* h, const uint8_t* idx, int32_t B, int32_t N, int32_t L, const int32_t* sites, int32_t S,
                     int32_t K, float* out) {
    if (!h) return PF_EINVAL;
    if (!sites) return fail(h, PF_EINVAL, "null buffer");
    return sites_impl(h, idx, B, N, L, sites, 0, S, K, out);
}

int pf_forward_windows(pf_handle_t* h, const uint8_t* idx, int32_t B, int32_t N, int32_t L, int32_t W, int32_t step, float* out,
                       int32_t S_cap) {
    if (!h) return PF_EINVAL;
    if (step < 1) return fail(h, PF_EINVAL, "windows need step >= 1 (got %d)", step);
    int rc = check_dims(h, B, N, L, L);
    if (rc) return rc;
    if (W < 1 || W > L) return fail(h, PF_EINVAL, "a site set needs 1 <= K <= L sites (got K=%d, L=%d)", W, L);
    const int S = pfsites::window_count(L, W, step);
    if (S < 0) return fail(h, PF_EINVAL, "bad window rule L=%d W=%d step=%d", L, W, step);
    if (S_cap < S) return fail(h, PF_EINVAL, "out holds %d windows, L=%d W=%d step=%d gives %d", S_cap, L, W, step, S);
    return sites_impl(h, idx, B, N, L, nullptr, step, S, W, out);
}

int pf_gather_taxa_device(pf_handle_t* h, const uint8_t* d_src, int32_t B, int32_t N, int32_t L, const int32_t* d_taxa, int32_t S,
                          int32_t M, uint8_t* d_dst) {
    if (!h) return PF_EINVAL;
    if (!d_src || !d_dst || !d_taxa) return fail(h, PF_EINVAL, "null buffer");
    if (B < 1 || N < 1 || L < 1 || S < 1 || M < 1) return fail(h, PF_EINVAL, "bad dimensions B=%d N=%d L=%d S=%d M=%d", B, N, L, S, M);
    size_t n = 0;
    if (!mul_size((size_t)B, (size_t)S, (size_t)M * L, &n) || !mul_size((size_t)S, (size_t)M, sizeof(int32_t), &n) ||
        !mul_size((size_t)B, (size_t)N, (size_t)L, &n))
        return fail(h, PF_EINVAL, "B=%d x S=%d taxon sets of %d x %d overflow the address space", B, S, M, L);
    HIPCHK(h, hipSetDevice(h->device));
    return launch_gather_taxa(h, d_src, B, N, L, d_taxa, 0, S, M, d_dst);
}

int pf_forward_taxa(pf_handle_t* h, const uint8_t* idx, int32_t B, int32_t N, int32_t L, const int32_t* taxa, int32_t S, int32_t M,
                    float* out) {
    if (!h) return PF_EINVAL;
    return taxa_impl(h, idx, B, N, L, taxa, S, M, out);
}

int pf_forward_leave_one_out(pf_handle_t* h, const uint8_t* idx, int32_t B, int32_t N, int32_t L, float* out, float* loo,
                             float* influence, float* shift, float* context) {
    if (!h) return PF_EINVAL;
    return loo_impl(h, idx, B, N, L, out, loo, influence, shift, context);
}

int pf_loo_stats_device(pf_handle_t* h, const float* d_full, const float* d_loo, int32_t B, int32_t N, float* d_influence,
                        float* d_shift, float* d_context) {
    if (!h) return PF_EINVAL;
    if (!d_full || !d_loo || !d_influence || !d_shift || !d_context) return fail(h, PF_EINVAL, "null buffer");
    if (B < 1 || N < 3 || N > 32767) return fail(h, PF_EINVAL, "bad dimensions B=%d N=%d (leave-one-out needs 3 <= N <= 32767)", B, N);
    size_t n = 0;
    if (!mul_size((size_t)B, (size_t)N, (size_t)(N - 1) * (N - 2) / 2 * sizeof(float), &n))
        return fail(h, PF_EINVAL, "B=%d x %d leave-one-out sets of %d sequences overflow the address space", B, N, N - 1);
    HIPCHK(h, hipSetDevice(h->device));
    return launch_loo_stats(h, d_full, d_loo, B, N, d_influence, d_shift, d_context);
}

int pf_forward_place(pf_handle_t* h, const uint8_t* idx, int32_t B, int32_t M, int32_t L, int32_t Q, float* out, float* base,
                     float* sets, float* place, float* disturb, float* shift, float* joint) {
    if (!h) return PF_EINVAL;
    return place_impl(h, idx, B, M, L, Q, out, base, sets, place, disturb, shift, joint);
}

int pf_place_stats_device(pf_handle_t* h, const float* d_whole, const float* d_base, const float* d_sets, int32_t B, int32_t N,
                          int32_t Q, float* d_place, float* d_disturb, float* d_shift, float* d_joint) {
    if (!h) return PF_EINVAL;
    if (!d_whole || !d_base || !d_sets || !d_place || !d_disturb || !d_shift || !d_joint) return fail(h, PF_EINVAL, "null buffer");
    if (B < 1 || N < 2 || Q < 1 || (int64_t)N + Q > 32767)
        return fail(h, PF_EINVAL, "bad dimensions B=%d N=%d Q=%d (placement needs N >= 2, Q >= 1, N + Q <= 32767)", B, N, Q);
    size_t n = 0;
    if (!mul_size((size_t)B, (size_t)Q, (size_t)(N + 1) * N / 2 * sizeof(float), &n) ||
        !mul_size((size_t)B, (size_t)(N + Q) * (N + Q - 1) / 2, sizeof(float), &n))
        return fail(h, PF_EINVAL, "B=%d x %d query sets of %d sequences overflow the address space", B, Q, N + 1);
    HIPCHK(h, hipSetDevice(h->device));
    return launch_place_stats(h, d_whole, d_base, d_sets, B, N, Q, d_place, d_disturb, d_shift, d_joint);
}

int pf_tile_groups(int32_t N, int32_t M) {
    const int64_t g = pftile::groups(N, M);
    return g < 0 ? PF_EINVAL : (int)g;
}

// ... 327 lines not shown
    HIPCHK(h, hipStreamSynchronize(h->stream));
    return PF_OK;
}
int pf_memcpy_d2h(pf_handle_t* h, void* dst, const void* src, size_t bytes) {
    if (!h) return PF_EINVAL;
    HIPCHK(h, hipMemcpyAsync(dst, src, bytes, hipMemcpyDeviceToHost, h->stream));
    HIPCHK(h, hipStreamSynchronize(h->stream));
    return check_bad_idx(h);
}

int pf_profile_reset(pf_handle_t* h) {
    if (!h) return PF_EINVAL;
    drain_profile(h);
    for (int i = 0; i < K_COUNT; ++i) { h->prof_n[i] = 0; h->prof_ms[i] = 0; }
    h->coll_calls = 0;
    h->rechecked = 0;
    h->nj_calls = 0;
    h->bionj_calls = 0;
    h->delta_calls = 0;
    h->bme_calls = 0;
    h->spr_calls = 0;
    h->sup_calls = 0;
    h->transfer_calls = 0;
    h->con_calls = 0;
    return PF_OK;
}

int pf_profile_get(pf_handle_t* h, const char* kernel, int64_t* launches, double* total_ms) {
    if (!h || !kernel) return PF_EINVAL;
    drain_profile(h);
    if (std::strcmp(kernel, "collectives") == 0) {
        if (launches) *launches = h->coll_calls;
        if (total_ms) *total_ms = 0.0;
        return PF_OK;
    }
    if (std::strcmp(kernel, "rechecked") == 0) {
        if (launches) *launches = h->rechecked;
        if (total_ms) *total_ms = 0.0;
        return PF_OK;
    }
    if (std::strcmp(kernel, "nj_joins") == 0) {
        if (launches) *launches = h->nj_calls;
        if (total_ms) *total_ms = 0.0;
        return PF_OK;
    }
    if (std::strcmp(kernel, "bionj_joins") == 0) {
        if (launches) *launches = h->bionj_calls;
        if (total_ms) *total_ms = 0.0;
        return PF_OK;
    }
    if (std::strcmp(kernel, "delta") == 0) {
        if (launches) *launches = h->delta_calls;
        if (total_ms) *total_ms = 0.0;
        return PF_OK;
    }
    if (std::strcmp(kernel, "bme_nni") == 0) {
        if (launches) *launches = h->bme_calls;
        if (total_ms) *total_ms = 0.0;
        return PF_OK;
    }
    if (std::strcmp(kernel, "bme_spr") == 0) {
        if (launches) *launches = h->spr_calls;
        if (total_ms) *total_ms = 0.0;
        return PF_OK;
    }
    if (std::strcmp(kernel, "join_supports") == 0) {
        if (launches) *launches = h->sup_calls;
        if (total_ms) *total_ms = 0.0;
        return PF_OK;
    }
    if (std::strcmp(kernel, "join_transfers") == 0) {
        if (launches) *launches = h->transfer_calls;
        if (total_ms) *total_ms = 0.0;
        return PF_OK;
    }
    if (std::strcmp(kernel, "join_consensus") == 0) {
        if (launches) *launches = h->con_calls;
        if (total_ms) *total_ms = 0.0;
        return PF_OK;
    }
    for (int i = 0; i < K_COUNT; ++i)
        if (std::strcmp(kernel, KNAMES[i]) == 0) {
            if (launches) *launches = h->prof_n[i];
            if (total_ms) *total_ms = h->prof_ms[i];
            return PF_OK;
        }
    return fail(h, PF_EINVAL, "unknown kernel '%s'", kernel);
}

int64_t pf_debug_read(pf_handle_t* h, const char* name, float* dst, int64_t cap) {
    if (!h || !name) return PF_EINVAL;
    if (std::strcmp(name, "phase_prof") == 0) {
        if (!h->phase_prof) return fail(h, PF_ESTATE, "phase_prof not enabled");
        unsigned long long v[8];
        hipStreamSynchronize(h->stream);
        if (hipMemcpy(v, h->phase_prof, 64, hipMemcpyDeviceToHost) != hipSuccess) return fail(h, PF_EHIP, "phase_prof copy");
        for (int i = 0; i < 8 && i < cap; ++i) dst[i] = (float)((double)v[i] * 1e-6);
        return 8;
    }
    if (std::strcmp(name, "f16_ranges") == 0) {
        if (dst && cap > 0) dst[0] = h->f16_ok ? 1.f : 0.f;
        if (dst && cap > 1) dst[1] = (float)h->f16_vmax_col;
        return 2;
    }
    auto it = h->taps.find(name);
    if (it == h->taps.end()) return fail(h, PF_ESTATE, "no tap '%s' (set debug_keep=1 and run a forward)", name);
    const int64_t n = (int64_t)it->second.size();
    if (dst) std::memcpy(dst, it->second.data(), (size_t)std::min(n, cap) * sizeof(float));
    return n;
}

int pf_device_info(pf_handle_t* h, char* name_out, size_t name_cap, int32_t* cu_count, uint64_t* hbm_bytes) {
    if (!h) return PF_EINVAL;
    if (name_out && name_cap) {
        char nm[256] = {0};
        snprintf(nm, sizeof nm, "%s", h->prop.name);
        if (!nm[0] && hipDeviceGetName(nm, (int)sizeof nm, h->device) != hipSuccess) nm[0] = 0;
        if (!nm[0]) snprintf(nm, sizeof nm, "AMD GPU");
        snprintf(name_out, name_cap, "%s (%s)", nm, h->prop.gcnArchName);
    }
    if (cu_count) *cu_count = h->prop.multiProcessorCount;
    if (hbm_bytes) *hbm_bytes = h->prop.totalGlobalMem;
    return PF_OK;
}

int pf_device_pci(pf_handle_t* h, int32_t* domain, int32_t* bus, int32_t* device) {
    if (!h) return PF_EINVAL;
    if (domain) *domain = h->prop.pciDomainID;
    if (bus) *bus = h->prop.pciBusID;
    if (device) *device = h->prop.pciDeviceID;
    return PF_OK;
}

int pf_forward_shards_emulated(pf_handle_t* h, const uint8_t* idx, int32_t B, int32_t N, int32_t L,
                               int32_t nshards, float* out) {
    if (!h) return PF_EINVAL;
    int rc = check_dims(h, B, N, L, L);
    if (rc) return rc;
    if (nshards < 1 || nshards > 64 || !idx || !out) return fail(h, PF_EINVAL, "bad shard count or null buffer");
    HIPCHK(h, hipSetDevice(h->device));
    if (const F64Path* f = f64_path_of(h, N, L)) return forward_shards_emulated_f64(h, *f, idx, B, N, L, nshards, out);
    if ((rc = ensure_pairs(h, N))) return rc;
    const int P = N * (N - 1) / 2;
    ShardStage stage(h);
    if ((rc = stage.upload(idx, B, N, L, nshards))) return rc;
    std::vector<ShardRun> runs;
    for (const ShardStage::Shard& s : stage.shards) {
        ShardRun r{{}, s.d_idx, nullptr, B, N, P, s.Lloc, L, tile_plan(h, P, s.Lloc), h->stream, {}};
        size_t off[WS_BUFS];
        char* ws = (char*)stage.alloc(workspace_bytes(h, B, P, r.Lloc, &r.w, off));
        r.d_out = (float*)stage.alloc((size_t)B * P * sizeof(float));
        if (!ws || !r.d_out) return fail(h, PF_ENOMEM, "shard workspace allocation failed");
        carve_workspace(ws, off, &r.w, B, r.Lloc);
        runs.push_back(r);
    }
    float* total = (float*)stage.alloc((size_t)B * P * SROW * sizeof(float));
    if (!total) return fail(h, PF_ENOMEM, "shard sum buffer");
    auto reduce = [&](bool site_sums) -> int {
        const size_t count = (size_t)B * P * (site_sums ? 1 : SROW);
        for (ShardRun& r : runs)
            if (!site_sums && (rc = launch_rowsum(h, r, &r.rs))) return rc;
        hipMemsetAsync(total, 0, count * sizeof(float), h->stream);
        for (ShardRun& r : runs) {
            hipLaunchKernelGGL(k_accumulate, dim3((unsigned)((count + 255) / 256)), dim3(256), 0, h->stream,
                               total, site_sums ? r.d_out : r.w.srow, count);
            r.rs = RowStats{total, 1, 0};
        }
        return PF_OK;
    };
    rc = schedule(h, runs.data(), runs.size(), reduce);
    if (!rc && (hipMemcpyAsync(out, total, (size_t)B * P * sizeof(float), hipMemcpyDeviceToHost, h->stream) != hipSuccess ||
                hipStreamSynchronize(h->stream) != hipSuccess))
        rc = fail(h, PF_EHIP, "result copy failed");
    return rc;
}

int pf_selftest(pf_handle_t* h, float* out) {
    if (!h || !out) return PF_EINVAL;
    float* d = nullptr;
    HIPCHK(h, hipMalloc((void**)&d, 2304 * sizeof(float)));
    hipLaunchKernelGGL(k_selftest, dim3(1), dim3(64), 0, h->stream, d);
    HIPCHK(h, hipGetLastError());
    HIPCHK(h, hipMemcpyAsync(out, d, 2304 * sizeof(float), hipMemcpyDeviceToHost, h->stream));
    HIPCHK(h, hipStreamSynchronize(h->stream));
    hipFree(d);
    return PF_OK;
}

struct pf_mha {
    pf_handle* h = nullptr;
    float* wfrag = nullptr;
    float* bias = nullptr;
    std::vector<DeviceBuffer*> buffers;
    Buffer<char> ws{buffers};
    Buffer<float> d_x{buffers}, d_y{buffers};
};

int pf_mha_create(pf_handle_t* h, const pf_mha_weights_t* w, pf_mha_t** out) {
    if (!h || !w || !out) return PF_EINVAL;
    if (w->n_heads != MHA_H || w->embed_dim != E)
        return fail(h, PF_EINVAL, "softmax attention kernels are specialised for embed_dim 64 / 4 heads, got %d / %d",
                    w->embed_dim, w->n_heads);
    const float* ws[4] = {w->wq, w->wk, w->wv, w->wo};
    const float* bs[4] = {w->bq, w->bk, w->bv, w->bo};
    std::vector<uint16_t> img((size_t)MHA_WTOTAL * 8);
    std::vector<float> bias(4 * E);
    for (int i = 0; i < 4; ++i) {
        if (!ws[i] || !bs[i]) return fail(h, PF_EINVAL, "pf_mha_create: NULL weight pointer");
        std::copy(bs[i], bs[i] + E, bias.begin() + i * E);
    }
    pack_frags(w->wq, E, E, E, img.data());
    pack_frags(w->wk, E, E, E, img.data() + (size_t)MHA_OFF_WK * 8);
    pack_frags(w->wv, E, E, E, img.data() + (size_t)MHA_OFF_WV * 8);
    pack_frags(w->wo, E, E, E, img.data() + (size_t)MHA_OFF_WO * 8);
    HIPCHK(h, hipSetDevice(h->device));
    pf_mha* m = new pf_mha();
    m->h = h;
    void* p = nullptr;
    if (hipMalloc(&p, img.size() * 2) != hipSuccess) { delete m; return fail(h, PF_ENOMEM, "pf_mha_create: hipMalloc failed"); }
    m->wfrag = (float*)p;
    if (hipMalloc(&p, bias.size() * 4) != hipSuccess) { hipFree(m->wfrag); delete m; return fail(h, PF_ENOMEM, "pf_mha_create: hipMalloc failed"); }
    m->bias = (float*)p;
    if (hipMemcpy(m->wfrag, img.data(), img.size() * 2, hipMemcpyHostToDevice) != hipSuccess ||
        hipMemcpy(m->bias, bias.data(), bias.size() * 4, hipMemcpyHostToDevice) != hipSuccess) {
        hipFree(m->wfrag); hipFree(m->bias); delete m;
        return fail(h, PF_EHIP, "pf_mha_create: weight upload failed");
    }
    *out = m;
    return PF_OK;
}

int pf_mha_destroy(pf_mha_t* m) {
    if (!m) return PF_OK;
    hipSetDevice(m->h->device);
    hipStreamSynchronize(m->h->stream);
    hipFree(m->wfrag); hipFree(m->bias);
    for (DeviceBuffer* b : m->buffers) b->release();
    delete m;
    return PF_OK;
}

int pf_mha_forward_device(pf_mha_t* m, const float* d_x, int32_t B, int32_t R, int32_t C, float* d_y) {
    if (!m || !d_x || !d_y) return PF_EINVAL;
    pf_handle* h = m->h;
    if (B < 1 || R < 1 || C < 1) return fail(h, PF_EINVAL, "pf_mha_forward: need B, R, C >= 1, got %d, %d, %d", B, R, C);
    const int64_t rows64 = (int64_t)B * R;
    const int ntiles = (C + 31) / 32;
    if (rows64 * MHA_H * ((ntiles + 3) / 4) > 0x7fffffffLL || rows64 * ntiles > 0x7fffffffLL)
        return fail(h, PF_EINVAL, "pf_mha_forward: B*R*C too large for one launch");
    const int rows = (int)rows64;
    HIPCHK(h, hipSetDevice(h->device));
    MhaArgs a;
    auto list = [&](auto& v) { pfspan::mha_arrays(v, a.qp, a.kp, a.vp, a.att, (size_t)rows, (size_t)MHA_H, (size_t)ntiles, (size_t)C, (size_t)E); };
    if (const int rc = m->ws.reserve(h, pfspan::measure(list, 256))) return rc;
    pfspan::carve(m->ws, list, 256);
    a.x = d_x; a.y = d_y;
    a.wfrag = (const frag_t*)m->wfrag;
    a.bias = m->bias;
    a.rows = rows; a.C = C; a.ntiles = ntiles;
    a.qscale = (float)(1.4426950408889634 / std::sqrt((double)MHA_D));
    const int cus = h->prop.multiProcessorCount > 0 ? h->prop.multiProcessorCount : 256;
    const int lin_tiles = rows * ntiles;
    const int g1 = std::max(1, std::min((lin_tiles + 3) / 4, cus * 3));
    {
        ProfScope ps(h, K_MHA_QKV);
        launch_mha_qkv(h->stream, (unsigned)g1, a);
    }
    HIPCHK(h, hipGetLastError());
    {
        ProfScope ps(h, K_MHA_ATTN);
        launch_mha_attn(h->stream, (unsigned)(rows * MHA_H * ((ntiles + 3) / 4)), a);
    }
    HIPCHK(h, hipGetLastError());
    const int64_t out_tiles = ((int64_t)rows * C + 31) / 32;
    const int g3 = (int)std::max<int64_t>(1, std::min<int64_t>((out_tiles + 3) / 4, cus * 8));
    {
        ProfScope ps(h, K_MHA_OUT);
        launch_mha_out(h->stream, (unsigned)g3, a);
    }
    HIPCHK(h, hipGetLastError());
    return PF_OK;
}

int pf_mha_forward(pf_mha_t* m, const float* x, int32_t B, int32_t R, int32_t C, float* y) {
    if (!m || !x || !y) return PF_EINVAL;
    pf_handle* h = m->h;
    if (B < 1 || R < 1 || C < 1) return fail(h, PF_EINVAL, "pf_mha_forward: need B, R, C >= 1, got %d, %d, %d", B, R, C);
    HIPCHK(h, hipSetDevice(h->device));
    const size_t bytes = (size_t)B * R * C * E * 4;
    int rc = m->d_x.reserve(h, bytes);
    if (rc || (rc = m->d_y.reserve(h, bytes))) return rc;
    HIPCHK(h, hipMemcpyAsync(m->d_x, x, bytes, hipMemcpyHostToDevice, h->stream));
    if ((rc = pf_mha_forward_device(m, m->d_x, B, R, C, m->d_y))) return rc;
    HIPCHK(h, hipMemcpyAsync(y, m->d_y, bytes, hipMemcpyDeviceToHost, h->stream));
    HIPCHK(h, hipStreamSynchronize(h->stream));
    return PF_OK;
}

}
```

Measured before the change: 579.0.

## Route main-kernel tiles over unique site columns for duplicate-heavy alignments

Adds a per-alignment plan kernel that splits alignments by how many unique site columns they have. Alignments whose unique count is at or below a threshold run the main block through a compact tiling over unique columns only. A follow-up stats launch (or a head-parts gather) then broadcasts the results back to the duplicate sites, while the other alignments take the original route. This avoids redundant per-site MFMA work on repeated columns, at the cost of extra launches, binary-search tile indexing and scatter passes.

```diff
diff --git a/phyloformer_amd/csrc/pf_device.hip.h b/phyloformer_amd/csrc/pf_device.hip.h
--- a/phyloformer_amd/csrc/pf_device.hip.h
+++ b/phyloformer_amd/csrc/pf_device.hip.h
@@ -328,31 +328,81 @@
     float* sitemap;
     const float* w;
     const int* srep;
+    const int* acount;
+    const int* alist;
+    const int* cpre;
+    const int* ulist;
+    const int* ucount;
+    float* term;
 };
 
-enum { MODE_FIRST = 0, MODE_MID = 1, MODE_LAST = 2, MODE_MID0 = 3, MODE_LAST_FOLD = 4 };
-
-struct TilePos { int b, kt, r0, l0; };
-template <bool FLAT>
+enum { MODE_FIRST = 0, MODE_MID = 1, MODE_LAST = 2, MODE_MID0 = 3, MODE_LAST_FOLD = 4, MODE_STATS = 5 };
+enum { ROUTE_ALL = 0, ROUTE_LIST = 1, ROUTE_COMPACT = 2 };
+
+struct TilePos { int b, kt, r0, l0, bi, K, nt; };
+__device__ __forceinline__ void compact_enter(const MainArgs& a, TilePos& q) {
+    q.b = a.alist[q.bi];
+    q.K = a.ucount[q.b];
+    q.nt = a.cpre[q.bi + 1] - a.cpre[q.bi];
+}
+template <bool FLAT, int ROUTE>
 __device__ __forceinline__ TilePos tile_pos(const MainArgs& a, int task, int ntiles) {
     TilePos q;
+    if (ROUTE == ROUTE_COMPACT) {
+        int lo = 0, hi = *a.acount - 1;
+        while (lo < hi) {
+            const int mid = (lo + hi + 1) >> 1;
+            if (a.cpre[mid] <= task) lo = mid; else hi = mid - 1;
+        }
+        q.bi = lo;
+        compact_enter(a, q);
+        q.kt = task - a.cpre[lo];
+        const CompactTile c = compact_tile(a.P, q.K, q.kt);
+        q.r0 = c.r0; q.l0 = c.u0;
+        return q;
+    }
+    if (ROUTE == ROUTE_LIST) {
+        q.bi = task / a.nt_aln;
+        q.kt = task - q.bi * a.nt_aln;
+        q.b = a.alist[q.bi];
+    } else {
     q.b = task / a.nt_aln;
     q.kt = task - q.b * a.nt_aln;
+    }
     if (FLAT) { const int tok0 = q.kt * 32; q.r0 = tok0 / a.Lloc; q.l0 = tok0 - q.r0 * a.Lloc; }
     else { q.r0 = q.kt / ntiles; q.l0 = (q.kt - q.r0 * ntiles) * 32; }
     return q;
 }
-template <bool FLAT>
+template <bool FLAT, int ROUTE>
 __device__ __forceinline__ TilePos tile_next(const MainArgs& a, TilePos q) {
+    if (ROUTE == ROUTE_COMPACT) {
+        if (++q.kt == q.nt) { q.bi = min(q.bi + 1, *a.acount - 1); compact_enter(a, q); q.kt = 0; q.r0 = 0; q.l0 = 0; return q; }
+        compact_next(q.K, &q.r0, &q.l0);
+        return q;
+    }
+    if (ROUTE == ROUTE_LIST) {
+        if (++q.kt == a.nt_aln) { q.bi = min(q.bi + 1, *a.acount - 1); q.b = a.alist[q.bi]; q.kt = 0; q.r0 = 0; q.l0 = 0; return q; }
+    } else
     if (++q.kt == a.nt_aln) { q.b++; q.kt = 0; q.r0 = 0; q.l0 = 0; return q; }
     q.l0 += 32;
     if (q.l0 >= a.Lloc) { q.l0 = FLAT ? q.l0 - a.Lloc : 0; q.r0++; }
     return q;
 }
-struct LanePos { size_t tok0; int toff, l, nvalid, wrap; bool valid, in_r1; };
-template <bool FLAT>
+struct LanePos { size_t tok0, tok; int toff, l, nvalid, wrap; bool valid, in_r1; };
+template <bool FLAT, int ROUTE>
 __device__ __forceinline__ LanePos lane_pos(const MainArgs& a, const TilePos& q, int t) {
     LanePos o;
+    if (ROUTE == ROUTE_COMPACT) {
+        o.nvalid = compact_nvalid(a.P, q.K, q.kt);
+        o.wrap = compact_wrap(a.P, q.K, q.r0, q.l0);
+        o.valid = t < o.nvalid;
+        o.toff = min(t, o.nvalid - 1);
+        o.in_r1 = o.toff >= o.wrap;
+        o.l = a.ulist[(size_t)q.b * a.Lloc + (q.l0 + o.toff - (o.in_r1 ? q.K : 0))];
+        o.tok0 = 0;
+        o.tok = ((size_t)q.b * a.P + q.r0 + (o.in_r1 ? 1 : 0)) * a.Lloc + o.l;
+        return o;
+    }
     o.tok0 = ((size_t)q.b * a.P + q.r0) * a.Lloc + q.l0;
     const int left = FLAT ? a.P * a.Lloc - q.kt * 32 : a.Lloc - q.l0;
     o.nvalid = min(32, left);
@@ -361,6 +411,7 @@
     o.toff = min(t, o.nvalid - 1);
     o.in_r1 = o.toff >= o.wrap;
     o.l = q.l0 + o.toff - (o.in_r1 ? a.Lloc : 0);
+    o.tok = o.tok0 + o.toff;
     return o;
 }
 __device__ __forceinline__ void part_range(int flat, int pr, int nparts, int P, int L, int slots_aln, long* first, int* count) {
@@ -382,23 +433,29 @@
     }
 }
 
-template <int MODE, bool FLAT, bool SITEMAP = false, bool WEIGHTED = false>
+template <int MODE, bool FLAT, bool SITEMAP = false, bool WEIGHTED = false, int ROUTE = ROUTE_ALL>
 __global__ void __launch_bounds__(MAIN_THREADS, MAIN_WAVES / 4) k_main(MainArgs a) {
     constexpr bool LAST = MODE == MODE_LAST || MODE == MODE_LAST_FOLD;
     constexpr bool FOLD = MODE == MODE_LAST_FOLD;
+    constexpr bool COMPACT = ROUTE == ROUTE_COMPACT;
+    constexpr bool STATS = MODE == MODE_STATS;
     static_assert(!SITEMAP || LAST, "the site map is the head's: last block only");
     static_assert(!WEIGHTED || (!SITEMAP && MODE != MODE_FIRST), "weighted launches: blocks' own modes, no site map");
+    static_assert(ROUTE == ROUTE_ALL || (!SITEMAP && !WEIGHTED && MODE != MODE_FIRST), "site-map, weighted and embedding launches are not routed");
+    static_assert(!STATS || ROUTE == ROUTE_LIST, "the statistics launch walks the split-route list in the original tiling");
+    static_assert(!COMPACT || FLAT, "the compact tiling has one instantiation");
     extern __shared__ __attribute__((aligned(16))) unsigned char smem[];
     lds_frag_t lw = (lds_frag_t)smem;
     lds_f32_t lc = (lds_f32_t)(smem + FRAG_END * 16);
 
+    if (ROUTE != ROUTE_ALL && *a.acount == 0) return;
     {
         const float cv = a.consts[min((int)threadIdx.x, CONST_LEN - 1)];
         if (FOLD) {
             image_to_lds<FRAG_W1, FRAG_W2>(a.wimg, smem);
             image_to_lds<FRAG_WO, FRAG_U + U_FRAGS>(a.wimg, smem);
         } else {
-            image_to_lds<(MODE == MODE_FIRST) ? FRAG_WV : 0, LAST ? FRAG_WV : FRAG_END>(a.wimg, smem);
+            image_to_lds<(MODE == MODE_FIRST || STATS) ? FRAG_WV : 0, LAST ? FRAG_WV : FRAG_END>(a.wimg, smem);
         }
         static_assert(CONST_LEN <= MAIN_THREADS, "one constant per thread");
         if (threadIdx.x < CONST_LEN) reinterpret_cast<float*>(smem + FRAG_END * 16)[threadIdx.x] = cv;
@@ -411,7 +468,7 @@
     const int t = lane & 31;
     const int h = lane >> 5;
     const int ntiles = (a.Lloc + 31) >> 5;
-    const int ntasks = a.B * a.nt_aln;
+    const int ntasks = COMPACT ? a.cpre[*a.acount] : (ROUTE == ROUTE_LIST ? *a.acount : a.B) * a.nt_aln;
     if (wave >= MAIN_WAVES / 2) __builtin_amdgcn_s_setprio(1);
     unsigned long long tacc[6] = {0, 0, 0, 0, 0, 0}, tprev = 0;
 #define PF_TICK(k) do { if (a.prof) { const unsigned long long tn_ = __builtin_amdgcn_s_memtime(); tacc[k] += tn_ - tprev; tprev = tn_; } } while (0)
@@ -433,16 +490,23 @@
         const int run = max(1, min(PF_RUN_MAX, ntasks / (nwaves * 8)));
         int run0 = (blockIdx.x * MAIN_WAVES + wave) * run;
         const int task0 = run0, task1 = ntasks;
-        TilePos cur = tile_pos<FLAT>(a, min(task0, ntasks - 1), ntiles);
+        TilePos cur = tile_pos<FLAT, ROUTE>(a, min(task0, ntasks - 1), ntiles);
         int frag_row = -1;
         frag_t mfr[4];
         f32x4 rqv = {0.f, 0.f, 0.f, 0.f};
         f32x4 px[8], pctx[8], pqr, pqc;
         int pri = 0, prj = 0;
         auto prefetch = [&](const TilePos& np) {
-            const LanePos nl = lane_pos<FLAT>(a, np, t);
+            const LanePos nl = lane_pos<FLAT, ROUTE>(a, np, t);
             const int ll = nl.l, pb = np.b;
-            const size_t tk = nl.tok0 + nl.toff;
+            const size_t tk = nl.tok;
+            if (STATS) {
+                const f32x4* xp = reinterpret_cast<const f32x4*>(
+                    a.x + (tk + (size_t)(long)(a.srep[(size_t)pb * a.Lloc + ll] - ll)) * 64 + 4 * h);
+#pragma unroll
+                for (int g = 0; g < 8; ++g) px[g] = xp[2 * g];
+                return;
+            }
             if (MODE == MODE_MID0) {
                 const uint8_t* ib = a.idx + (size_t)pb * a.N * a.Lloc + ll;
                 const int pp = np.r0 + (nl.in_r1 ? 1 : 0);
@@ -469,13 +533,13 @@
             const int b = cur.b;
             const int row = b * a.P + cur.r0;
             int ntask = task + 1;
-            TilePos nxt = tile_next<FLAT>(a, cur);
+            TilePos nxt = tile_next<FLAT, ROUTE>(a, cur);
             if (ntask == run0 + run) {
                 run0 += nwaves * run;
                 ntask = run0;
-                if (ntask < task1) nxt = tile_pos<FLAT>(a, ntask, ntiles);
-            }
-            const LanePos lp = lane_pos<FLAT>(a, cur, t);
+                if (ntask < task1) nxt = tile_pos<FLAT, ROUTE>(a, ntask, ntiles);
+            }
+            const LanePos lp = lane_pos<FLAT, ROUTE>(a, cur, t);
             const bool straddle = lp.wrap < 32;
             int ai = 0, aj = 0;
             if (MODE == MODE_FIRST) { const int pp = cur.r0 + (lp.in_r1 ? 1 : 0); ai = a.pair_i[pp]; aj = a.pair_j[pp]; }
@@ -487,16 +551,22 @@
                 rqv = *(const_f32x4_t)(unsigned long long)(a.rq + (size_t)__builtin_amdgcn_readfirstlane(r) * 4);
                 frag_row = r;
             };
-            if (MODE != MODE_FIRST && row != frag_row) load_mfr(row);
+            if (MODE != MODE_FIRST && !STATS && row != frag_row) load_mfr(row);
             const bool valid = lp.valid;
             const int lc_ = lp.l;
-            const size_t tok = lp.tok0 + lp.toff;
+            const size_t tok = lp.tok;
             float x[32];
             float zh[4] = {0.f, 0.f, 0.f, 0.f};
             float wt = 1.f;
             if (WEIGHTED && LAST) wt = a.w[(size_t)b * a.Lloc + lc_];
 
-            if (MODE == MODE_FIRST) {
+            if (STATS) {
+#pragma unroll
+                for (int g = 0; g < 8; ++g)
+#pragma unroll
+                    for (int i = 0; i < 4; ++i) x[4 * g + i] = px[g][i];
+                if (ntask < task1) prefetch(nxt);
+            } else if (MODE == MODE_FIRST) {
                 const int ri = residue(a.idx[((size_t)b * a.N + ai) * a.Lloc + lc_]);
                 const int rj = residue(a.idx[((size_t)b * a.N + aj) * a.Lloc + lc_]);
                 const f32x4* ti = reinterpret_cast<const f32x4*>(a.table + ri * 64 + 4 * h);
@@ -671,12 +741,16 @@
 
             if (!LAST && !(a.ablate & 4)) {
                 frag_t wl[8];
+                if (!COMPACT) {
 #pragma unroll
                 for (int i = WVLO_LDS; i < 8; ++i) wl[i] = a.wv_lo[i * 64 + lane];
+                }
                 if (WEIGHTED) wt = a.w[(size_t)b * a.Lloc + lc_];
                 __builtin_amdgcn_sched_barrier(0);
-                {
-                    const size_t stok = valid ? tok : a.trash_tok + t;
+                if (!STATS || a.store_x_last) {
+                    bool keep = valid;
+                    if (STATS) keep = valid && a.srep[(size_t)b * a.Lloc + lc_] != lc_;
+                    const size_t stok = keep ? tok : a.trash_tok + t;
                     f32x4* xo = reinterpret_cast<f32x4*>(a.x + stok * 64 + 4 * h);
 #pragma unroll
                     for (int g = 0; g < 8; ++g) {
@@ -684,7 +758,7 @@
                         xo[2 * g] = u;
                     }
                 }
-                if (a.ablate & 32) { cur = nxt; task = ntask; continue; }
+                if (COMPACT || (a.ablate & 32)) { cur = nxt; task = ntask; continue; }
                 f32x16 va[3];
                 {
                     float xn[32];
@@ -761,12 +835,13 @@
                     z = pair_sum(z) + lc[CONST_HB];
                 }
                 const float spz = softplus20(z);
+                if (COMPACT) { if (valid && h == 0) a.term[tok] = spz; }
                 const long slot0 = (long)b * a.slots_aln + cur.kt + (FLAT ? cur.r0 : 0);
-                for (int part = 0; part < (straddle ? 2 : 1); ++part) {
+                for (int part = 0; part < (COMPACT ? 0 : straddle ? 2 : 1); ++part) {
                     const float so = half32_sum((valid && lp.in_r1 == (part == 1)) ? (WEIGHTED ? wt * spz : spz) : 0.f);
                     if (lane == 0) a.outpart[slot0 + part] = so;
                 }
-                if (SITEMAP && valid && h == 0) a.sitemap[lp.tok0 + lp.toff] = spz;
+                if (SITEMAP && valid && h == 0) a.sitemap[tok] = spz;
                 if (!FOLD && a.store_x_last && valid) {
                     f32x4* xo = reinterpret_cast<f32x4*>(a.x + tok * 64 + 4 * h);
 #pragma unroll
@@ -1039,6 +1114,52 @@
     out[pr] = acc * (wst ? wst[(size_t)(pr / P) * 4 + 1] : inv_L_total);
 }
 
+__global__ void __launch_bounds__(64) k_main_plan(const int* ucount, int* plan, int B, int P, int Lloc, int mode) {
+    const int lane = threadIdx.x;
+    int* const flist = plan + 4;
+    int* const slist = flist + B;
+    int* const cpre = slist + B;
+    int nf = 0, ns = 0, tiles = 0;
+    for (int b0 = 0; b0 < B; b0 += 64) {
+        const int b = b0 + lane;
+        const int K = b < B ? ucount[b] : 0;
+        const bool split = b < B && main_dedup_split(K, Lloc, mode);
+        const bool fused = b < B && !split;
+        const unsigned long long ms = __ballot(split), mf = __ballot(fused), below = (1ull << lane) - 1ull;
+        int incl = split ? compact_tiles(P, K) : 0;
+        const int mine = incl;
+#pragma unroll
+        for (int d = 1; d < 64; d <<= 1) { const int o = __shfl_up(incl, d); if (lane >= d) incl += o; }
+        if (split) { const int i = ns + __popcll(ms & below); slist[i] = b; cpre[i] = tiles + incl - mine; }
+        if (fused) flist[nf + __popcll(mf & below)] = b;
+        ns += __popcll(ms);
+        nf += __popcll(mf);
+        tiles += __shfl(incl, 63);
+    }
+    if (lane == 0) { plan[0] = nf; plan[1] = ns; plan[2] = tiles; plan[3] = 0; cpre[ns] = tiles; }
+}
+
+template <bool FLAT>
+__global__ void __launch_bounds__(256) k_head_parts(MainArgs a) {
+    const int ns = *a.acount;
+    if (ns == 0) return;
+    const int lane = threadIdx.x & 63, t = lane & 31;
+    const int ntiles = (a.Lloc + 31) >> 5;
+    const int ntasks = ns * a.nt_aln;
+    for (int task = blockIdx.x * 4 + (threadIdx.x >> 6); task < ntasks; task += gridDim.x * 4) {
+        const TilePos cur = tile_pos<FLAT, ROUTE_LIST>(a, task, ntiles);
+        const LanePos lp = lane_pos<FLAT, ROUTE_LIST>(a, cur, t);
+        const size_t row0 = ((size_t)cur.b * a.P + cur.r0 + (lp.in_r1 ? 1 : 0)) * a.Lloc;
+        const float spz = a.term[row0 + a.srep[(size_t)cur.b * a.Lloc + lp.l]];
+        const bool straddle = lp.wrap < 32;
+        const long slot0 = (long)cur.b * a.slots_aln + cur.kt + (FLAT ? cur.r0 : 0);
+        for (int part = 0; part < (straddle ? 2 : 1); ++part) {
+            const float so = half32_sum((lp.valid && lp.in_r1 == (part == 1)) ? spz : 0.f);
+            if (lane == 0) a.outpart[slot0 + part] = so;
+        }
+    }
+}
+
 struct SiteClassArgs {
     const uint8_t* idx;
     int* srep;
diff --git a/phyloformer_amd/csrc/pf_layout.h b/phyloformer_amd/csrc/pf_layout.h
--- a/phyloformer_amd/csrc/pf_layout.h
+++ b/phyloformer_amd/csrc/pf_layout.h
@@ -41,4 +41,41 @@
 
 constexpr int PAIRTAB_ROWS = 22 * 22, PAIRTAB_W = 72;
 
+#if defined(__HIPCC__)
+#define PF_HD __host__ __device__
+#else
+#define PF_HD
+#endif
+#ifndef PF_MAIN_DEDUP_NUM
+#define PF_MAIN_DEDUP_NUM 17
+#define PF_MAIN_DEDUP_DEN 20
+#endif
+constexpr int MAIN_DEDUP_NUM = PF_MAIN_DEDUP_NUM, MAIN_DEDUP_DEN = PF_MAIN_DEDUP_DEN;
+PF_HD inline bool main_dedup_split(int K, int L, int mode) {
+    return mode == 2 || (mode == 1 && (long)K * MAIN_DEDUP_DEN <= (long)L * MAIN_DEDUP_NUM);
 }
+PF_HD inline int compact_tiles(int P, int K) { return K >= 32 ? (int)(((long)P * K + 31) >> 5) : P; }
+PF_HD inline int compact_nvalid(int P, int K, int kt) {
+    const long left = K >= 32 ? (long)P * K - (long)kt * 32 : K;
+    return left < 32 ? (int)left : 32;
+}
+PF_HD inline int compact_wrap(int P, int K, int r0, int u0) {
+    return (K >= 32 && r0 + 1 < P && K - u0 < 32) ? K - u0 : 32;
+}
+struct CompactTile { int r0, u0, nvalid, wrap; };
+PF_HD inline CompactTile compact_tile(int P, int K, int kt) {
+    CompactTile c;
+    if (K >= 32) { const long tok0 = (long)kt * 32; c.r0 = (int)(tok0 / K); c.u0 = (int)(tok0 - (long)c.r0 * K); }
+    else { c.r0 = kt; c.u0 = 0; }
+    c.nvalid = compact_nvalid(P, K, kt);
+    c.wrap = compact_wrap(P, K, c.r0, c.u0);
+    return c;
+}
+PF_HD inline void compact_next(int K, int* r0, int* u0) {
+    if (K < 32) { ++*r0; return; }
+    *u0 += 32;
+    if (*u0 >= K) { *u0 -= K; ++*r0; }
+}
+PF_HD inline int main_plan_ints(int B) { return 4 + 3 * B + 1; }
+
+}
diff --git a/phyloformer_amd/csrc/pf_lib.hip b/phyloformer_amd/csrc/pf_lib.hip
--- a/phyloformer_amd/csrc/pf_lib.hip
+++ b/phyloformer_amd/csrc/pf_lib.hip
@@ -191,6 +191,7 @@
     bool colstats_ring = true;
     bool materialize_x0 = false;
     bool site_dedup = true;
+    int main_dedup = 1;
     float* first_consts = nullptr;
     float* first_img = nullptr;
     std::vector<BlockDev> blk;
@@ -473,6 +474,7 @@
 struct Workspace {
     float *x, *qrow, *qcol, *srow, *mrow, *part, *ctx, *mfrag, *spart, *outpart, *rq;
     int *srep, *ulist, *ucount;
+    int* plan;
     int G;
     int sub, S, fine;
     int nparts() const { return fine ? G * S : G; }
@@ -498,7 +500,7 @@
     off[8] = o; o = align_up(o + (size_t)B * slots * SROW * 4, 256);
     off[9] = o; o = align_up(o + (size_t)B * slots * 4, 256);
     off[10] = o; o = align_up(o + (size_t)B * P * 4 * 4, 256);
-    off[11] = o; o = align_up(o + ((size_t)B * Lloc * 2 + B) * sizeof(int), 256);
+    off[11] = o; o = align_up(o + ((size_t)B * Lloc * 2 + B + main_plan_ints(B)) * sizeof(int), 256);
     return o;
 }
 void carve_workspace(char* ws, const size_t off[WS_BUFS], Workspace* w, int B, int Lloc) {
@@ -511,6 +513,7 @@
     w->rq = (float*)(ws + off[10]);
     const size_t nsite = (size_t)B * std::max(Lloc, 1);
     w->srep = (int*)(ws + off[11]); w->ulist = w->srep + nsite; w->ucount = w->ulist + nsite;
+    w->plan = w->ucount + B;
 }
 
 int ensure_workspace(pf_handle* h, int B, int P, int Lloc, Workspace* w, bool second = false) {
@@ -532,7 +535,7 @@
     pf_handle* h; int kid; hipEvent_t a{}, b{};
     bool on;
     ProfScope(pf_handle* h_, int kid_) : h(h_), kid(kid_) {
-        on = h->profile && (!h->profile_main_only || kid_ == K_MAIN);
+        on = kid_ >= 0 && h->profile && (!h->profile_main_only || kid_ == K_MAIN);
         if (on) { a = get_event(h); b = get_event(h); hipEventRecord(a, h->cur); }
     }
     ~ProfScope() {
@@ -574,14 +577,38 @@
     return PF_OK;
 }
 
-template <int MODE, bool SITEMAP = false, bool WEIGHTED = false>
+template <int MODE, bool SITEMAP = false, bool WEIGHTED = false, int ROUTE = ROUTE_ALL>
 int launch_main(pf_handle* h, const MainArgs& a, int kid) {
     const long ntasks = (long)a.B * a.nt_aln;
     const int cus = std::max(1, h->prop.multiProcessorCount - (h->reducing ? h->reserve_cus : 0));
     const int grid = (int)std::max<long>(1, std::min<long>(cus, (ntasks + MAIN_WAVES - 1) / MAIN_WAVES));
     ProfScope ps(h, kid);
-    if (a.flat) hipLaunchKernelGGL((k_main<MODE, true, SITEMAP, WEIGHTED>), dim3(grid), dim3(MAIN_THREADS), MAIN_LDS_BYTES, h->cur, a);
-    else hipLaunchKernelGGL((k_main<MODE, false, SITEMAP, WEIGHTED>), dim3(grid), dim3(MAIN_THREADS), MAIN_LDS_BYTES, h->cur, a);
+    if constexpr (ROUTE == ROUTE_COMPACT)
+        hipLaunchKernelGGL((k_main<MODE, true, SITEMAP, WEIGHTED, ROUTE>), dim3(grid), dim3(MAIN_THREADS), MAIN_LDS_BYTES, h->cur, a);
+    else if (a.flat) hipLaunchKernelGGL((k_main<MODE, true, SITEMAP, WEIGHTED, ROUTE>), dim3(grid), dim3(MAIN_THREADS), MAIN_LDS_BYTES, h->cur, a);
+    else hipLaunchKernelGGL((k_main<MODE, false, SITEMAP, WEIGHTED, ROUTE>), dim3(grid), dim3(MAIN_THREADS), MAIN_LDS_BYTES, h->cur, a);
+    HIPCHK(h, hipGetLastError());
+    return PF_OK;
+}
+
+template <int MODE>
+int launch_main_routed(pf_handle* h, const MainArgs& m, const int* plan) {
+    constexpr bool last = MODE == MODE_LAST || MODE == MODE_LAST_FOLD;
+    int rc;
+    MainArgs f = m;
+    f.acount = plan; f.alist = plan + 4;
+    if ((rc = launch_main<MODE, false, false, ROUTE_LIST>(h, f, -1))) return rc;
+    MainArgs c = m;
+    c.acount = plan + 1; c.alist = plan + 4 + m.B; c.cpre = c.alist + m.B;
+    c.term = m.spart;
+    c.prof = nullptr;
+    if ((rc = launch_main<MODE, false, false, ROUTE_COMPACT>(h, c, -1))) return rc;
+    if (!last) return launch_main<MODE_STATS, false, false, ROUTE_LIST>(h, c, -1);
+    const long ntasks = (long)m.B * m.nt_aln;
+    const int cus = std::max(1, h->prop.multiProcessorCount - (h->reducing ? h->reserve_cus : 0));
+    const int grid = (int)std::max<long>(1, std::min<long>(8L * cus, (ntasks + 3) / 4));
+    if (m.flat) hipLaunchKernelGGL(k_head_parts<true>, dim3(grid), dim3(256), 0, h->cur, c);
+    else hipLaunchKernelGGL(k_head_parts<false>, dim3(grid), dim3(256), 0, h->cur, c);
     HIPCHK(h, hipGetLastError());
     return PF_OK;
 }
@@ -598,6 +625,7 @@
     float* d_smap = nullptr;
     const float* d_w = nullptr;
     const float* d_wst = nullptr;
+    bool routed = false;
 };
 
 int zero_fill(pf_handle* h, float* p, size_t n) {
@@ -618,6 +646,7 @@
     m.prof = h->phase_prof_last ? nullptr : h->phase_prof;
     m.w = r.d_w;
     m.srep = r.w.srep;
+    m.ulist = r.w.ulist; m.ucount = r.w.ucount;
     return m;
 }
 
@@ -625,11 +654,18 @@
     return !h->materialize_x0 && !h->embed_mfma && h->n_blocks > 1;
 }
 
-int launch_site_classes(pf_handle* h, const uint8_t* d_idx, int B, int N, int Lloc, int* srep, int* ulist, int* ucount) {
+bool routes_main(const pf_handle* h, const ShardRun& r) {
+    return h->main_dedup != 0 && !r.d_smap && !r.d_w && x0_on_the_fly(h) && r.Lloc > 0;
+}
+
+int launch_site_classes(pf_handle* h, const uint8_t* d_idx, int B, int N, int Lloc, int* srep, int* ulist, int* ucount,
+                        int* plan = nullptr, int P = 0) {
     if (!Lloc) return PF_OK;
     SiteClassArgs a{d_idx, srep, ulist, ucount, N, Lloc, h->site_dedup ? 1 : 0};
     ProfScope ps(h, K_SITE_CLASSES);
     hipLaunchKernelGGL(k_site_classes, dim3(B), dim3(SC_THREADS), 0, h->cur, a);
+    HIPCHK(h, hipGetLastError());
+    if (plan) hipLaunchKernelGGL(k_main_plan, dim3(1), dim3(64), 0, h->cur, ucount, plan, B, P, Lloc, h->main_dedup);
     HIPCHK(h, hipGetLastError());
     return PF_OK;
 }
@@ -740,10 +776,15 @@
     MainArgs m = main_args(h, r);
     m.wimg = reinterpret_cast<const frag_t*>(d.wimg);
     m.consts = d.consts;
+    const int* plan = r.routed ? w.plan : nullptr;
+    const int kid = plan ? -1 : K_MAIN;
+    {
+    ProfScope ps(h, plan ? K_MAIN : -1);
     if (k + 1 < h->n_blocks) {
         m.wv_lo = reinterpret_cast<const frag_t*>(h->blk[k + 1].wv_lo);
         const bool first = k == 0 && x0_on_the_fly(h);
-        if (r.d_w) rc = first ? launch_main<MODE_MID0, false, true>(h, m, K_MAIN) : launch_main<MODE_MID, false, true>(h, m, K_MAIN);
+        if (plan) rc = first ? launch_main_routed<MODE_MID0>(h, m, plan) : launch_main_routed<MODE_MID>(h, m, plan);
+        else if (r.d_w) rc = first ? launch_main<MODE_MID0, false, true>(h, m, K_MAIN) : launch_main<MODE_MID, false, true>(h, m, K_MAIN);
         else rc = first ? launch_main<MODE_MID0>(h, m, K_MAIN) : launch_main<MODE_MID>(h, m, K_MAIN);
         if (rc) return rc;
     } else {
@@ -752,18 +793,21 @@
         m.sitemap = r.d_smap;
         if (!h->head_fold) {
             if ((rc = r.d_w      ? launch_main<MODE_LAST, false, true>(h, m, K_MAIN)
-                      : r.d_smap ? launch_main<MODE_LAST, true>(h, m, K_MAIN) : launch_main<MODE_LAST>(h, m, K_MAIN))) return rc;
+                      : r.d_smap ? launch_main<MODE_LAST, true>(h, m, K_MAIN)
+                      : plan && !h->debug_keep ? launch_main_routed<MODE_LAST>(h, m, plan) : launch_main<MODE_LAST>(h, m, kid))) return rc;
         } else {
             if ((rc = r.d_w      ? launch_main<MODE_LAST_FOLD, false, true>(h, m, K_MAIN)
-                      : r.d_smap ? launch_main<MODE_LAST_FOLD, true>(h, m, K_MAIN) : launch_main<MODE_LAST_FOLD>(h, m, K_MAIN)))
+                      : r.d_smap ? launch_main<MODE_LAST_FOLD, true>(h, m, K_MAIN)
+                      : plan     ? launch_main_routed<MODE_LAST_FOLD>(h, m, plan) : launch_main<MODE_LAST_FOLD>(h, m, K_MAIN)))
                 return rc;
             if (h->debug_keep) {
                 MainArgs md = m;
                 md.outpart = w.spart;
                 md.prof = nullptr;
-                if ((rc = r.d_w ? launch_main<MODE_LAST, false, true>(h, md, K_MAIN) : launch_main<MODE_LAST>(h, md, K_MAIN))) return rc;
+                if ((rc = r.d_w ? launch_main<MODE_LAST, false, true>(h, md, K_MAIN) : launch_main<MODE_LAST>(h, md, kid))) return rc;
             }
         }
+    }
     }
     if (h->debug_keep && (rc = save_tap(h, "x" + std::to_string(k + 1), w.x, (size_t)B * P * Lloc * 64))) return rc;
     return PF_OK;
@@ -798,7 +842,8 @@
     int rc;
     for (ShardRun* r = runs; r != end; ++r) {
         h->cur = r->stream;
-        if ((rc = launch_site_classes(h, r->d_idx, r->B, r->N, r->Lloc, r->w.srep, r->w.ulist, r->w.ucount))) return rc;
+        if ((rc = launch_site_classes(h, r->d_idx, r->B, r->N, r->Lloc, r->w.srep, r->w.ulist, r->w.ucount,
+                                      r->routed ? r->w.plan : nullptr, r->P))) return rc;
         if ((rc = phase_first(h, *r))) return rc;
         r->rs = first_stats(h, *r);
     }
@@ -832,6 +877,7 @@
                         tile_plan(h, P, Lloc), h->stream, {}};
         if (d_smap) r[i].d_smap = d_smap + (size_t)b0 * P * Lloc;
         if (d_w) { r[i].d_w = d_w + (size_t)b0 * Lloc; r[i].d_wst = d_wst + (size_t)b0 * pfw::WST; }
+        r[i].routed = routes_main(h, r[i]);
         if ((rc = ensure_workspace(h, nb, P, Lloc, &r[i].w, i == 1))) return rc;
         b0 += nb;
     }
@@ -2277,6 +2323,7 @@
     else if (k == "force_rccl") h->force_rccl = value != 0;
     else if (k == "colstats_ring") h->colstats_ring = value != 0;
     else if (k == "site_dedup") h->site_dedup = value != 0;
+    else if (k == "main_dedup") h->main_dedup = value <= 0 ? 0 : (value >= 2 ? 2 : 1);
     else if (k == "precise") h->precise = value < 0 ? -1 : (value != 0);
     else if (k == "recheck_above") h->recheck_above = value > 0 ? (double)value : 0.0;
     else if (k == "precise_ffn_valu") h->precise_ffn_valu = value != 0;
@@ -2910,6 +2957,7 @@
         r.d_out = (float*)stage.alloc((size_t)B * P * sizeof(float));
         if (!ws || !r.d_out) return fail(h, PF_ENOMEM, "shard workspace allocation failed");
         carve_workspace(ws, off, &r.w, B, r.Lloc);
+        r.routed = routes_main(h, r);
         runs.push_back(r);
     }
     float* total = (float*)stage.alloc((size_t)B * P * SROW * sizeof(float));
```

Result: faster. 659.8, median of 6 (+14.0%).
